# maxpit/human-pose-estimation

Measured on AMD Instinct MI355X. Metric: images/sec (224x224, batch 256/GPU), higher is better.
Workload: dtype f32; 1 GPU; batch=256/GPU 224x224x3 synthetic images, fp32 ResNet-50 v1 + 3-iter regressor + SMPL LBS at all 3 stages (configs[1] at batch 256; the BASELINE metric batch); global_batch=256, parallelism=dp1 (batch shard, replicated weights), regressor=synthetic 'survey' variant, input=float32 images resident in HBM

## Files before the change

human-pose-estimation_amd/_lib.py:

```python
from __future__ import annotations

import ctypes as C
import os

import numpy as np

_HERE = os.path.dirname(os.path.abspath(__file__))
LIB_PATH = os.path.join(_HERE, "lib", "libhpe_hip.so")

NUM_CONV = 53
NUM_DENSE = 3
NUM_CRITIC_DENSE = 9
NUM_VERTS = 6890
THETA_DIM = 85
FEATURE_DIM = 2048


class HpeError(RuntimeError):
    pass


class HpeConfig(C.Structure):
    _fields_ = [
        ("struct_size", C.c_int),
# ... 122 lines not shown
    r = HpeConvRoute(struct_size=C.sizeof(HpeConvRoute))
    check(lib.hpe_debug_conv_route(C.byref(cfg), int(idx), int(B), int(concurrent), int(residual), int(workspace), C.byref(r)))
    return r


ENCODER_PACKINGS = ("w", "w_split", "wino_u", "wino4_u", "stem_w", "scale", "shift", "w_dual", "w_dual_split", "shift_dual", "dxw", "flat")

OUTPUT_FIELDS = ("verts", "joints", "cams", "theta", "J_transformed", "kp2d", "verts2d", "Rs")


class HpeOutputs(C.Structure):
    _fields_ = [(n, C.c_void_p) for n in OUTPUT_FIELDS]


REDUCE_FN = C.CFUNCTYPE(C.c_int, C.c_void_p, C.c_void_p, C.c_longlong, C.c_void_p)

_PROTOS = {
    "hpe_last_error": (C.c_char_p, []),
    "hpe_version": (C.c_char_p, []),
    "hpe_conv_layer_name": (C.c_char_p, [C.c_int]),
    "hpe_bn_layer_name": (C.c_char_p, [C.c_int]),
    "hpe_conv_layer_geometry": (C.c_int, [C.c_int, C.POINTER(C.c_int)]),
    "hpe_config_init": (None, [C.POINTER(HpeConfig)]),
    "hpe_create": (C.c_int, [C.POINTER(HpeConfig), C.POINTER(C.c_void_p)]),
    "hpe_destroy": (C.c_int, [C.c_void_p]),
    "hpe_load_smpl": (C.c_int, [C.c_void_p, C.POINTER(HpeSmplModel)]),
    "hpe_load_conv": (C.c_int, [C.c_void_p, C.c_int] + [C.c_void_p] * 6),
    "hpe_load_dense": (C.c_int, [C.c_void_p, C.c_int, C.c_void_p, C.c_void_p]),
    "hpe_load_mean_theta": (C.c_int, [C.c_void_p, C.c_void_p]),
    "hpe_finalize": (C.c_int, [C.c_void_p]),
    "hpe_forward": (C.c_int, [C.c_void_p, C.c_void_p, C.c_int, C.POINTER(HpeOutputs), C.c_int, C.c_void_p]),
    "hpe_forward_pipelined": (C.c_int, [C.c_void_p, C.c_void_p, C.c_int, C.POINTER(HpeOutputs), C.c_int, C.c_void_p]),
    "hpe_join": (C.c_int, [C.c_void_p, C.c_void_p]),
    "hpe_tail": (C.c_int, [C.c_void_p, C.c_void_p, C.c_int, C.POINTER(HpeOutputs), C.c_int, C.c_void_p]),
    "hpe_tail_stream": (C.c_void_p, [C.c_void_p]),
    "hpe_encoder": (C.c_int, [C.c_void_p, C.c_void_p, C.c_int, C.c_void_p, C.c_void_p]),
    "hpe_regress_stage": (C.c_int, [C.c_void_p, C.c_void_p, C.c_void_p, C.c_int, C.c_void_p, C.c_void_p]),
    "hpe_smpl": (C.c_int, [C.c_void_p, C.c_void_p, C.c_int, C.POINTER(HpeOutputs), C.c_void_p]),
    "hpe_smpl_backward": (C.c_int, [C.c_void_p, C.c_void_p, C.c_int, C.POINTER(HpeOutputs), C.c_void_p, C.c_void_p]),
    "hpe_orth_proj": (C.c_int, [C.c_void_p, C.c_void_p, C.c_int, C.c_int, C.c_void_p, C.c_void_p]),
    "hpe_reproject_vertices": (C.c_int, [C.c_void_p, C.c_void_p, C.c_int, C.c_int, C.c_float, C.c_float, C.c_void_p, C.c_void_p]),
    "hpe_preprocess_u8": (C.c_int, [C.c_void_p, C.c_int, C.c_int, C.c_int, C.c_void_p, C.POINTER(C.c_int), C.c_void_p]),
    "hpe_preprocess_u8_batch": (C.c_int, [C.c_void_p, C.POINTER(C.c_longlong), C.POINTER(C.c_int), C.c_int, C.c_int, C.c_void_p, C.POINTER(C.c_int),
                                          C.c_void_p, C.c_void_p]),
    "hpe_augment_plan": (C.c_int, [C.c_int, C.c_void_p, C.c_void_p, C.c_void_p, C.c_void_p, C.c_void_p, C.c_int, C.c_void_p, C.c_void_p, C.c_void_p]),
    "hpe_augment_batch": (C.c_int, [C.c_void_p, C.c_void_p, C.c_void_p, C.c_void_p, C.c_void_p, C.c_int, C.c_void_p, C.c_void_p, C.c_void_p, C.c_void_p]),
    "hpe_adam_advance": (C.c_int, [C.c_void_p, C.c_double, C.c_double, C.c_double, C.c_void_p]),
    "hpe_adam_apply": (C.c_int, [C.c_void_p, C.c_void_p, C.c_void_p, C.c_void_p, C.c_longlong, C.c_void_p, C.c_float, C.c_float, C.c_float, C.c_void_p]),
    "hpe_adam_set_step": (C.c_int, [C.c_void_p, C.c_longlong, C.c_double, C.c_double, C.c_void_p]),
    "hpe_debug_adam_power": (C.c_int, [C.c_double, C.c_longlong, C.POINTER(C.c_double)]),
    "hpe_jpeg_info": (C.c_int, [C.c_int, C.c_void_p, C.c_void_p, C.c_void_p]),
    "hpe_jpeg_decode": (C.c_int, [C.c_int, C.c_void_p, C.c_void_p, C.c_void_p, C.c_int, C.c_void_p, C.c_longlong, C.c_void_p, C.c_void_p, C.c_void_p]),
    "hpe_jpeg_backend": (C.c_int, [C.c_void_p, C.c_void_p, C.c_int, C.c_void_p, C.c_longlong, C.c_void_p, C.c_longlong, C.c_void_p, C.c_longlong,
                                   C.c_void_p]),
    "hpe_jpeg_encode_layout": (C.c_int, [C.c_int, C.c_void_p, C.c_void_p, C.c_int, C.c_int, C.c_int, C.c_void_p, C.c_void_p]),
    "hpe_jpeg_forward": (C.c_int, [C.c_void_p, C.c_void_p, C.c_int, C.c_void_p, C.c_longlong, C.c_void_p, C.c_longlong, C.c_void_p]),
    "hpe_jpeg_entropy_encode": (C.c_int, [C.c_void_p, C.c_int, C.c_void_p, C.c_longlong, C.c_int, C.c_int, C.c_int, C.c_int, C.c_void_p, C.c_longlong,
                                          C.c_void_p, C.c_void_p]),
    "hpe_png_backend": (C.c_int, [C.c_void_p, C.c_void_p, C.c_int, C.c_void_p, C.c_longlong, C.c_void_p, C.c_longlong, C.c_void_p, C.c_longlong,
                                  C.c_void_p]),
    "hpe_png_filter": (C.c_int, [C.c_void_p, C.c_void_p, C.c_int, C.c_void_p, C.c_longlong, C.c_void_p, C.c_longlong, C.c_void_p]),
    "hpe_draw_panels": (C.c_int, [C.c_void_p] * 6 + [C.c_int, C.c_int, C.c_int, C.c_void_p, C.c_void_p]),
    "hpe_draw_skeleton": (C.c_int, [C.c_void_p] * 4 + [C.c_int, C.c_int, C.c_int, C.c_int, C.c_int, C.c_void_p]),
    "hpe_get_original": (C.c_int, [C.c_void_p, C.c_void_p, C.c_int, C.c_int, C.c_int, C.POINTER(C.c_int), C.c_float, C.c_int, C.c_void_p, C.POINTER(C.c_float), C.c_void_p, C.c_void_p, C.c_void_p]),
    "hpe_kp_loss": (C.c_int, [C.c_void_p, C.c_void_p, C.c_int, C.c_int, C.c_void_p, C.c_void_p]),
    "hpe_kp_loss_backward": (C.c_int, [C.c_void_p, C.c_void_p, C.c_int, C.c_int, C.c_void_p, C.c_void_p, C.c_void_p]),
    "hpe_mesh_loss": (C.c_int, [C.c_void_p, C.c_void_p, C.c_void_p, C.c_int, C.c_int, C.c_int, C.c_int, C.c_void_p, C.c_void_p]),
    "hpe_mesh_loss_grad": (C.c_int, [C.c_void_p, C.c_void_p, C.c_void_p, C.c_int, C.c_int, C.c_int, C.c_int, C.c_void_p, C.c_void_p, C.c_void_p,
                                     C.c_void_p, C.c_void_p]),
    "hpe_val_losses": (C.c_int, [C.c_void_p, C.c_void_p, C.c_void_p, C.POINTER(C.c_void_p), C.POINTER(C.c_void_p), C.c_int, C.c_int, C.c_int,
                                 C.c_int, C.c_int, C.c_int, C.c_void_p, C.c_void_p]),
    "hpe_eval_scores": (C.c_int, [C.POINTER(C.c_void_p), C.c_void_p, C.c_int, C.c_void_p, C.c_void_p, C.POINTER(C.c_void_p), C.c_int, C.c_int, C.c_int,
                                  C.c_int, C.c_int, C.c_int, C.c_void_p, C.c_void_p, C.c_void_p, C.c_void_p]),
    "hpe_critic_layer_name": (C.c_char_p, [C.c_int]),
    "hpe_critic_layer_shape": (C.c_int, [C.c_int, C.POINTER(C.c_int)]),
    "hpe_load_critic": (C.c_int, [C.c_void_p, C.POINTER(HpeCriticModel)]),
    "hpe_critic": (C.c_int, [C.c_void_p, C.c_void_p, C.c_int, C.c_void_p, C.c_int, C.c_void_p, C.c_int, C.c_void_p, C.c_void_p, C.c_void_p]),
    "hpe_critic_backward": (C.c_int, [C.c_void_p, C.c_void_p, C.c_int, C.c_void_p, C.c_int, C.c_void_p, C.c_int, C.c_void_p, C.c_void_p,
                                      C.c_void_p, C.c_void_p, C.c_void_p, C.c_void_p]),
    "hpe_critic_param_floats": (C.c_int, []),
    "hpe_critic_param_offset": (C.c_int, [C.c_int, C.c_int]),
    "hpe_critic_weight_grad_ws_floats": (C.c_longlong, [C.c_int]),
    "hpe_critic_reserve": (C.c_int, [C.c_void_p, C.c_int]),
    "hpe_critic_weight_grad": (C.c_int, [C.c_void_p, C.c_void_p, C.c_int, C.c_void_p, C.c_int, C.c_void_p, C.c_int, C.c_void_p, C.c_void_p,
                                         C.c_void_p, C.c_void_p, C.c_void_p, C.c_int, C.c_void_p, C.c_void_p]),
    "hpe_critic_get_params": (C.c_int, [C.c_void_p, C.c_void_p, C.c_void_p]),
    "hpe_critic_set_params_dev": (C.c_int, [C.c_void_p, C.c_void_p, C.c_void_p]),
    "hpe_regressor_param_floats": (C.c_int, []),
    "hpe_regressor_param_offset": (C.c_int, [C.c_int, C.c_int]),
    "hpe_regressor_get_params": (C.c_int, [C.c_void_p, C.c_void_p, C.c_void_p]),
    "hpe_regressor_set_params_dev": (C.c_int, [C.c_void_p, C.c_void_p, C.c_void_p]),
    "hpe_regressor_forward_train": (C.c_int, [C.c_void_p, C.c_void_p, C.c_int, C.c_void_p, C.c_void_p, C.c_void_p]),
    "hpe_regressor_backward": (C.c_int, [C.c_void_p, C.c_void_p, C.c_int, C.c_void_p, C.c_void_p, C.c_void_p, C.c_void_p, C.c_void_p]),
    "hpe_encoder_param_floats": (C.c_int, []),
    "hpe_encoder_param_offset": (C.c_int, [C.c_int, C.c_int]),
    "hpe_encoder_train_reserve": (C.c_int, [C.c_void_p, C.c_int]),
    "hpe_encoder_train_ws_floats": (C.c_longlong, [C.c_int]),
    "hpe_encoder_wg_slices": (C.c_int, [C.c_int, C.c_int]),
    "hpe_encoder_forward_train": (C.c_int, [C.c_void_p, C.c_void_p, C.c_int, C.c_void_p, C.c_void_p]),
    "hpe_encoder_backward": (C.c_int, [C.c_void_p, C.c_void_p, C.c_int, C.c_void_p, C.c_void_p, C.c_void_p]),
    "hpe_encoder_get_params": (C.c_int, [C.c_void_p, C.c_void_p, C.c_void_p]),
    "hpe_encoder_set_params": (C.c_int, [C.c_void_p, C.c_void_p]),
    "hpe_encoder_set_params_dev": (C.c_int, [C.c_void_p, C.c_void_p, C.c_void_p]),
    "hpe_debug_encoder_packing_bytes": (C.c_longlong, [C.c_void_p, C.c_int, C.c_int]),
    "hpe_debug_encoder_packing": (C.c_int, [C.c_void_p, C.c_int, C.c_int, C.c_void_p, C.c_void_p]),
    "hpe_debug_conv_backward": (C.c_int, [C.c_void_p, C.c_int, C.c_void_p, C.c_void_p, C.c_void_p, C.c_int, C.c_void_p, C.c_void_p, C.c_void_p]),
    "hpe_debug_maxpool_backward": (C.c_int, [C.c_void_p, C.c_void_p, C.c_int, C.c_int, C.c_int, C.c_void_p, C.c_void_p]),
    "hpe_debug_avgpool_backward": (C.c_int, [C.c_void_p, C.c_int, C.c_int, C.c_int, C.c_void_p, C.c_void_p]),
    "hpe_debug_encoder_stash": (C.c_int, [C.c_void_p, C.c_int, C.c_void_p, C.c_void_p]),
    "hpe_debug_encoder_stash_batch": (C.c_int, [C.c_void_p]),
    "hpe_encoder_train_reserve_mixed": (C.c_int, [C.c_void_p, C.c_int]),
    "hpe_encoder_train_ws_floats_mixed": (C.c_longlong, [C.c_int]),
    "hpe_encoder_forward_train_mixed": (C.c_int, [C.c_void_p, C.c_void_p, C.c_int, C.c_void_p, C.c_void_p]),
    "hpe_encoder_backward_mixed": (C.c_int, [C.c_void_p, C.c_void_p, C.c_int, C.c_void_p, C.c_void_p, C.c_void_p]),
    "hpe_debug_conv_backward_mixed": (C.c_int, [C.c_void_p, C.c_int, C.c_void_p, C.c_void_p, C.c_void_p, C.c_int, C.c_void_p, C.c_void_p, C.c_void_p]),
    "hpe_debug_maxpool_backward_mixed": (C.c_int, [C.c_void_p, C.c_void_p, C.c_int, C.c_int, C.c_int, C.c_void_p, C.c_void_p]),
    "hpe_debug_avgpool_backward_mixed": (C.c_int, [C.c_void_p, C.c_int, C.c_int, C.c_int, C.c_void_p, C.c_void_p]),
    "hpe_debug_encoder_stash_mixed": (C.c_int, [C.c_void_p, C.c_int, C.c_void_p, C.c_void_p]),
    "hpe_debug_encoder_stash_batch_mixed": (C.c_int, [C.c_void_p]),
    "hpe_encoder_stat_floats": (C.c_int, []),
    "hpe_encoder_stat_offset": (C.c_int, [C.c_int, C.c_int]),
    "hpe_encoder_train_reserve_batchnorm": (C.c_int, [C.c_void_p, C.c_int]),
    "hpe_encoder_train_ws_floats_batchnorm": (C.c_longlong, [C.c_int]),
    "hpe_debug_encoder_bn_slices": (C.c_int, [C.c_int, C.c_int]),
    "hpe_encoder_forward_batchnorm": (C.c_int, [C.c_void_p, C.c_void_p, C.c_int, C.c_void_p, C.c_void_p]),
    "hpe_encoder_backward_batchnorm": (C.c_int, [C.c_void_p, C.c_void_p, C.c_int, C.c_void_p, C.c_void_p, C.c_void_p]),
    "hpe_encoder_get_stats": (C.c_int, [C.c_void_p, C.c_void_p, C.c_void_p]),
    "hpe_encoder_update_stats": (C.c_int, [C.c_void_p, C.c_void_p, C.c_double, C.c_int, C.c_void_p]),
    "hpe_encoder_set_stats_dev": (C.c_int, [C.c_void_p, C.c_void_p, C.c_void_p]),
    "hpe_debug_conv_batchnorm": (C.c_int, [C.c_void_p, C.c_int, C.c_void_p, C.c_int, C.c_void_p, C.c_int, C.c_void_p, C.c_void_p, C.c_void_p, C.c_void_p]),
    "hpe_debug_conv_backward_batchnorm": (C.c_int, [C.c_void_p, C.c_int, C.c_void_p, C.c_void_p, C.c_void_p, C.c_void_p, C.c_int, C.c_void_p, C.c_void_p,
                                                    C.c_void_p]),
    "hpe_debug_encoder_stash_raw": (C.c_int, [C.c_void_p, C.c_int, C.c_void_p, C.c_void_p]),
    "hpe_debug_encoder_batch_stats": (C.c_int, [C.c_void_p, C.c_void_p, C.c_void_p]),
    "hpe_encoder_set_reduce": (C.c_int, [C.c_void_p, REDUCE_FN, C.c_void_p, C.c_int]),
    "hpe_debug_bn_sums": (C.c_int, [C.c_void_p, C.c_int, C.c_void_p, C.c_int, C.c_void_p, C.c_void_p]),
    "hpe_debug_bn_finish": (C.c_int, [C.c_void_p, C.c_int, C.c_void_p, C.c_longlong, C.c_void_p, C.c_int, C.c_void_p, C.c_int, C.c_void_p, C.c_void_p,
                                      C.c_void_p]),
    "hpe_debug_bn_backward_sums": (C.c_int, [C.c_void_p, C.c_int, C.c_void_p, C.c_void_p, C.c_void_p, C.c_int, C.c_void_p, C.c_longlong, C.c_void_p,
                                             C.c_void_p]),
    "hpe_debug_bn_backward_finish": (C.c_int, [C.c_void_p, C.c_int, C.c_void_p, C.c_void_p, C.c_void_p, C.c_void_p, C.c_int, C.c_void_p, C.c_void_p,
                                               C.c_longlong, C.c_void_p, C.c_void_p, C.c_void_p]),
    "hpe_device_status": (C.c_int, [C.c_void_p, C.c_void_p]),
    "hpe_debug_conv": (C.c_int, [C.c_void_p, C.c_int, C.c_void_p, C.c_int, C.c_void_p, C.c_int, C.c_void_p, C.c_void_p]),
    "hpe_debug_chain": (C.c_int, [C.c_void_p, C.c_int, C.c_void_p, C.c_void_p, C.c_int, C.c_void_p, C.c_void_p, C.POINTER(C.c_int), C.c_void_p]),
    "hpe_debug_stem": (C.c_int, [C.c_void_p, C.c_void_p, C.c_int, C.c_int, C.c_void_p, C.c_void_p]),
    "hpe_debug_gemm": (C.c_int, [C.c_void_p, C.c_void_p, C.c_void_p, C.c_int, C.c_int, C.c_int, C.c_int, C.c_int, C.c_void_p, C.c_int, C.c_void_p, C.c_void_p]),
    "hpe_debug_gemm_ex": (C.c_int, [C.c_void_p, C.POINTER(HpeDebugGemm), C.c_void_p]),
    "hpe_debug_gemm_check": (C.c_int, [C.POINTER(HpeDebugGemm), C.c_int, C.c_int]),
    "hpe_debug_gemm_launch": (C.c_int, [C.c_void_p, C.POINTER(HpeDebugGemm), C.c_int, C.c_int, C.c_void_p]),
    "hpe_debug_conv_route": (C.c_int, [C.POINTER(HpeConfig), C.c_int, C.c_int, C.c_int, C.c_int, C.c_int, C.POINTER(HpeConvRoute)]),
    "hpe_debug_conv_stream1x1": (C.c_int, [C.POINTER(HpeConfig), C.c_int, C.c_int, C.c_int, C.c_int]),
    "hpe_debug_dual": (C.c_int, [C.c_void_p, C.c_int, C.c_void_p, C.c_void_p, C.c_int, C.c_void_p, C.c_void_p]),
    "hpe_debug_maxpool": (C.c_int, [C.c_void_p, C.c_int, C.c_int, C.c_int, C.c_void_p, C.c_void_p]),
    "hpe_debug_avgpool": (C.c_int, [C.c_void_p, C.c_int, C.c_int, C.c_int, C.c_void_p, C.c_void_p]),
    "hpe_debug_joint_regress": (C.c_int, [C.c_void_p, C.c_void_p, C.c_int, C.c_int, C.c_void_p, C.c_void_p]),
    "hpe_enable_timing": (C.c_int, [C.c_void_p, C.c_int]),
    "hpe_get_timings": (C.c_int, [C.c_void_p, C.POINTER(C.c_float)]),
    "hpe_get_span_stats": (C.c_int, [C.c_void_p, C.POINTER(C.c_float), C.POINTER(C.c_int)]),
    "hpe_get_loss_timings": (C.c_int, [C.c_void_p, C.POINTER(C.c_float)]),
    "hpe_debug_set_loss_counter": (C.c_int, [C.c_void_p, C.c_void_p]),
    "hpe_get_conv_timings": (C.c_int, [C.c_void_p, C.POINTER(C.c_float)]),
    "hpe_render_params_init": (None, [C.POINTER(HpeRenderParams)]),
    "hpe_renderer_create": (C.c_int, [C.c_int, C.c_void_p, C.c_int, C.c_int, C.c_int, C.POINTER(C.c_void_p)]),
    "hpe_renderer_destroy": (C.c_int, [C.c_void_p]),
    "hpe_render": (C.c_int, [C.c_void_p, C.c_void_p, C.c_void_p, C.c_int, C.c_int, C.c_int, C.c_void_p, C.POINTER(HpeRenderParams), C.c_void_p,
                             C.c_void_p]),
    "hpe_debug_render_ids": (C.c_int, [C.c_void_p, C.c_void_p, C.c_void_p, C.c_int, C.c_int, C.c_int, C.POINTER(HpeRenderParams), C.c_void_p,
                                       C.c_void_p, C.c_void_p]),
    "hpe_debug_render_vertices": (C.c_int, [C.c_void_p, C.c_void_p, C.c_void_p, C.c_int, C.c_int, C.c_int, C.POINTER(HpeRenderParams),
                                            C.c_void_p, C.c_void_p]),
}

_lib = None


def load():
    global _lib
    if _lib is not None:
        return _lib
    if not os.path.exists(LIB_PATH):
        raise HpeError(
            "%s not found: build it with `python -c 'import __graft_entry__ as g; g.build()'` "
            "(hipcc --offload-arch=gfx950).  There is no CPU fallback." % LIB_PATH
        )
    try:
        import torch
    except Exception:
        pass
    lib = C.CDLL(LIB_PATH, mode=C.RTLD_GLOBAL)
    for name, (res, args) in _PROTOS.items():
        fn = getattr(lib, name)
        fn.restype = res
        fn.argtypes = args
    _lib = lib
    return lib


def declared_symbols():
    return sorted(_PROTOS)


def check(rc):
    if rc != 0:
        msg = load().hpe_last_error()
        raise HpeError("libhpe_hip error %d: %s" % (rc, msg.decode() if msg else "?"))


def f32(a):
    arr = np.ascontiguousarray(a, dtype=np.float32)
    return arr, arr.ctypes.data_as(C.c_void_p)
```

human-pose-estimation_amd/build.py:

```python
from __future__ import annotations

import os
import shutil
import subprocess
import sys

HERE = os.path.dirname(os.path.abspath(__file__))
CSRC = os.path.join(HERE, "csrc")
LIBDIR = os.path.join(HERE, "lib")
LIB = os.path.join(LIBDIR, "libhpe_hip.so")
SOURCES = ["conv_gemm.hip", "conv_gemm_f32s.hip", "conv_stream_f32s.hip", "conv_gemm_bf16.hip", "conv_gemm_bf16_p8.hip", "conv_chain_bf16.hip", "conv_chain_f32.hip", "conv3_halo_bf16.hip", "conv_wino.hip", "conv_wino4.hip", "stem_fused.hip", "encoder_ops.hip", "smpl.hip", "losses.hip", "prepost.hip", "render.hip", "hpe_plan.hip", "hpe_finalize.hip", "hpe_encoder.hip", "hpe_api.hip", "hpe_render_api.hip", "smpl_bwd.hip", "critic.hip", "critic_train.hip", "regressor_train.hip", "augment.hip", "encoder_train.hip", "encoder_grad.hip", "encoder_grad_bf16.hip", "encoder_repack.hip", "encoder_bn.hip", "jpeg_entropy.hip", "jpeg_decode.hip", "jpeg_huffman_enc.hip", "jpeg_encode.hip", "png_decode.hip", "png_encode.hip", "draw.hip", "adam.hip", "eval_scores.hip"]
CFLAGS = ["--offload-arch=gfx950", "-O3", "-std=c++17", "-fPIC", "-fvisibility=hidden", "-fno-fast-math"]


def _hipcc():
    for cand in (os.environ.get("HIPCC"), shutil.which("hipcc"), "/opt/rocm/bin/hipcc"):
        if cand and os.path.exists(cand):
            return cand
    raise RuntimeError("hipcc not found (set HIPCC or install ROCm under /opt/rocm)")


def _deps():
    return [os.path.join(CSRC, f) for f in os.listdir(CSRC) if f.endswith(".h")] + [os.path.join(HERE, "..", "include", "hpe.h")]


def _obj_stale(src, obj):
    if not os.path.exists(obj):
        return True
    t = os.path.getmtime(obj)
    return any(os.path.getmtime(d) > t for d in [src] + _deps() if os.path.exists(d))


def _flags_now():
    return " ".join(CFLAGS + os.environ.get("HPE_EXTRA_FLAGS", "").split())


def built_flags():
    tag = os.path.join(LIBDIR, "obj", "flags.txt")
    return open(tag).read() if os.path.exists(tag) else ""


def _stale():
    if not os.path.exists(LIB):
        return True
    if built_flags() != _flags_now():
        return True
    t = os.path.getmtime(LIB)
    deps = [os.path.join(CSRC, f) for f in os.listdir(CSRC)] + [os.path.join(HERE, "..", "include", "hpe.h")]
    return any(os.path.getmtime(d) > t for d in deps if os.path.exists(d))


def build(force=False, verbose=False):
    if not force and not _stale():
        return LIB
    os.makedirs(LIBDIR, exist_ok=True)
    objdir = os.path.join(LIBDIR, "obj")
    os.makedirs(objdir, exist_ok=True)
    extra = os.environ.get("HPE_EXTRA_FLAGS", "").split()
    tag = os.path.join(objdir, "flags.txt")
    flags_now = _flags_now()
    if force or not os.path.exists(tag) or open(tag).read() != flags_now:
        for f in os.listdir(objdir):
            os.remove(os.path.join(objdir, f))
    hipcc = _hipcc()
    jobs = []
    for s in SOURCES:
        src = os.path.join(CSRC, s)
        if not os.path.exists(src):
            continue
        obj = os.path.join(objdir, s.replace(".hip", ".o"))
        jobs.append((src, obj))

    def compile_one(job):
        src, obj = job
        if not _obj_stale(src, obj):
            return None
        cmd = [hipcc] + CFLAGS + extra + ["-c", "-o", obj + ".tmp%d" % os.getpid(), src]
        if verbose:
            print(" ".join(cmd), file=sys.stderr)
        r = subprocess.run(cmd, capture_output=True, text=True)
        if r.returncode != 0:
            return "hipcc failed on %s:\n%s%s" % (os.path.basename(src), r.stdout, r.stderr)
        os.replace(obj + ".tmp%d" % os.getpid(), obj)
        return None

    from concurrent.futures import ThreadPoolExecutor

    with ThreadPoolExecutor(max_workers=min(len(jobs), max(1, (os.cpu_count() or 2) - 1))) as ex:
        errs = [e for e in ex.map(compile_one, jobs) if e]
    if errs:
        raise RuntimeError("\n".join(errs))
    open(tag, "w").write(flags_now)
    tmp = LIB + ".tmp%d" % os.getpid()
    cmd = [hipcc, "--offload-arch=gfx950", "-shared", "-fPIC", "-o", tmp] + [o for _, o in jobs]
    r = subprocess.run(cmd, capture_output=True, text=True)
    if r.returncode != 0:
        raise RuntimeError("link failed:\n" + r.stdout + r.stderr)
    os.replace(tmp, LIB)
    return LIB


if __name__ == "__main__":
    print(build(force="--force" in sys.argv, verbose=True))
```

human-pose-estimation_amd/csrc/conv_stream_f32s.hip:

```cpp
#include <hip/hip_runtime.h>
#include <stdint.h>

#include "bf16_split.h"
#include "conv_gemm_common.h"
#include "gemm_contract.h"
#include "hpe_internal.h"
#include "lds_dma.h"

namespace {

constexpr int SBM = 32, SBN = 128, SNW = 4;

template <int K, bool DUAL>
__global__ __launch_bounds__(64 * SNW, 2) void conv_stream_f32s_kernel(GemmArgs p, int walkers) {
    constexpr bool RES = !DUAL;
    constexpr int NRES = RES ? SBM / (64 * SNW / (SBN / 4)) : 0;
    constexpr int KS = K / 16;
    constexpr int CH = K / 8;
    constexpr int RAW_BYTES = SBM * K * 4;
    constexpr int PLANE_BYTES = SBM * K * 2;
    constexpr int EP_BYTES = SBM * (SBN + 4) * 4;
    constexpr int WORK_BYTES = 3 * PLANE_BYTES > EP_BYTES ? 3 * PLANE_BYTES : EP_BYTES;
    constexpr int AP = RAW_BYTES / 1024 / SNW;
    constexpr int UN = SBM * CH / (64 * SNW);
    constexpr int NPASS = SBM / (64 * SNW / (SBN / 4));
    static_assert(K == 64 || K == 128, "K = 64 or 128");
    static_assert(!DUAL || K == 128, "dual: two sources of 64");
    static_assert(AP >= 1 && UN >= 1 && NPASS == 4, "tile geometry");

    __shared__ __attribute__((aligned(16))) float lds[WORK_BYTES / 4];
    __shared__ __attribute__((aligned(16))) float raw_lds[2 * RAW_BYTES / 4];
    char* const work = reinterpret_cast<char*>(lds);
    char* const raw = reinterpret_cast<char*>(raw_lds);

    const int bid = blockIdx.x;
    const int j = bid >> 3;
    const int slice = j % p.n_ntiles;
    const int walker = (j / p.n_ntiles) * 8 + (bid & 7);
    if (walker >= walkers || walker >= p.n_mtiles) return;
    const int n0 = slice * SBN;
    const int cnt = (p.n_mtiles - walker + walkers - 1) / walkers;

    const int t = threadIdx.x;
    const int lane = t & 63;
    const int wave = __builtin_amdgcn_readfirstlane(t >> 6);
    const int hi = lane >> 5;

    bf16x8 wreg[KS][3];
    {
        const __bf16* wsrc = reinterpret_cast<const __bf16*>(p.w) + (size_t)(n0 + 32 * wave + (lane & 31)) * p.ldw + 8 * hi;
#pragma unroll
        for (int q = 0; q < KS; ++q)
#pragma unroll
            for (int pc = 0; pc < 3; ++pc) wreg[q][pc] = *reinterpret_cast<const bf16x8*>(wsrc + pc * p.w_piece + 16 * q);
    }
    const int ncol = n0 + 32 * wave + (lane & 31);
    const float sc0 = p.scale[ncol], sh0 = p.shift[ncol];

    int dma_row[AP], dma_col[AP];
#pragma unroll
    for (int i = 0; i < AP; ++i) {
        const int s = (SNW * i + wave) * 64 + lane;
        dma_row[i] = s / (K / 4);
        dma_col[i] = (s % (K / 4)) * 4;
    }
    int sp_src[UN], sp_dst[UN];
#pragma unroll
    for (int u = 0; u < UN; ++u) {
        const int un = t + 64 * SNW * u;
        const int r = un / CH, c = un % CH;
        sp_src[u] = r * (K * 4) + c * 32;
        sp_dst[u] = r * (K * 2) + ((c ^ ((r / (16 / CH)) & (CH - 1))) << 4);
    }
    const int a_row = (lane & 31) * (K * 2);
    const int a_x = ((lane & 31) / (16 / CH)) & (CH - 1);
    const int r_row = t >> 5;
    const float* const res_col = RES ? p.res + n0 + (t & 31) * 4 : nullptr;

    auto issue_tile = [&](int m0, int buf, f32x4 (&rnext)[NPASS]) {
        asm volatile("" ::: "memory");
#pragma unroll
        for (int i = 0; i < AP; ++i) {
            int m = m0 + dma_row[i];
            m = m < p.M ? m : p.M - 1;
            const float* src = p.x + ((size_t)m * p.lda + dma_col[i]);
            if (DUAL && dma_col[i] >= 64) src = p.x2 + ((size_t)m * p.Cin + (dma_col[i] - 64));
            dma16(src, raw + buf * RAW_BYTES + (SNW * i + wave) * 1024);
        }
        asm volatile("" ::: "memory");
#pragma unroll
        for (int pass = 0; pass < NRES; ++pass) {
            int m = m0 + pass * 8 + r_row;
            m = m < p.M ? m : p.M - 1;
            rnext[pass] = HPE_RES_LOAD(reinterpret_cast<const f32x4*>(res_col + (size_t)m * p.ldres));
        }
        asm volatile("" ::: "memory");
    };

    auto tile_step = [&](int k, int buf, f32x4 (&rcur)[NPASS], f32x4 (&rnext)[NPASS]) {
        const int m0 = (walker + k * walkers) * SBM;
        const int m0n = k + 1 < cnt ? m0 + walkers * SBM : m0;
        wait_counts<NRES + NPASS>();
        bare_barrier();
        const unsigned rb = (unsigned)(uintptr_t)(const __attribute__((address_space(3))) char*)(raw + buf * RAW_BYTES);
#pragma unroll
        for (int u = 0; u < UN; ++u) {
            f32x4 lo, up;
            asm volatile("ds_read_b128 %0, %2\n\tds_read_b128 %1, %2 offset:16\n\ts_waitcnt lgkmcnt(0)" : "=&v"(lo), "=&v"(up) : "v"(rb + sp_src[u]) : "memory");
            bf16x8 h0, h1, h2;
            bf16_split3_cast<8>([&](int e) { return e < 4 ? lo[e] : up[e - 4]; }, h0, h1, h2);
            *reinterpret_cast<bf16x8*>(work + sp_dst[u]) = h0;
            *reinterpret_cast<bf16x8*>(work + PLANE_BYTES + sp_dst[u]) = h1;
            *reinterpret_cast<bf16x8*>(work + 2 * PLANE_BYTES + sp_dst[u]) = h2;
        }
        lds_barrier();
        issue_tile(m0n, buf ^ 1, rnext);

        f32x16 acc[1][1], acx;
#pragma unroll
        for (int e = 0; e < 16; ++e) acc[0][0][e] = acx[e] = 0.f;
#pragma unroll
        for (int q = 0; q < KS; ++q) {
            const int off = a_row + (((2 * q + hi) ^ a_x) << 4);
            const bf16x8 a0 = *reinterpret_cast<const bf16x8*>(work + off);
            const bf16x8 a1 = *reinterpret_cast<const bf16x8*>(work + PLANE_BYTES + off);
            const bf16x8 a2 = *reinterpret_cast<const bf16x8*>(work + 2 * PLANE_BYTES + off);
            acx = __builtin_amdgcn_mfma_f32_32x32x16_bf16(a2, wreg[q][0], acx, 0, 0, 0);
            acx = __builtin_amdgcn_mfma_f32_32x32x16_bf16(a1, wreg[q][1], acx, 0, 0, 0);
            acx = __builtin_amdgcn_mfma_f32_32x32x16_bf16(a0, wreg[q][2], acx, 0, 0, 0);
            acx = __builtin_amdgcn_mfma_f32_32x32x16_bf16(a1, wreg[q][0], acx, 0, 0, 0);
            acx = __builtin_amdgcn_mfma_f32_32x32x16_bf16(a0, wreg[q][1], acx, 0, 0, 0);
            acc[0][0] = __builtin_amdgcn_mfma_f32_32x32x16_bf16(a0, wreg[q][0], acc[0][0], 0, 0, 0);
        }
        acc[0][0] += acx;
        wait_counts<AP + NRES, 0>();
        bare_barrier();
        conv_epilogue<SBM, SBN, 1, SNW, true>(p, lds, acc, m0, n0, t, lane, 0, wave, rcur, RES, sc0, sh0);
    };

    f32x4 ra[NPASS], rb[NPASS];
    issue_tile(walker * SBM, 0, ra);
    wait_counts<0>();
    for (int k = 0; k < cnt; k += 2) {
        tile_step(k, 0, ra, rb);
        if (k + 1 < cnt) tile_step(k + 1, 1, rb, ra);
    }
    wait_counts<0>();
}

int device_cus() {
    static int n = 0;
    if (n == 0) {
        int dev = 0, v = 0;
        if (hipGetDevice(&dev) == hipSuccess && hipDeviceGetAttribute(&v, hipDeviceAttributeMultiprocessorCount, dev) == hipSuccess && v > 0) n = v;
        else n = 256;
    }
    return n;
}

}

bool hpe_stream_f32s_supported(int M, int N, int K) { return M > 0 && (K == 64 || K == 128) && N >= SBN && N % SBN == 0; }

bool hpe_stream_f32s_dual_supported(int M, int N, int K1, int K2, int stride, int Hi, int Ho) {
    return K1 == 64 && K2 == 64 && stride == 1 && Hi == Ho && hpe_stream_f32s_supported(M, N, K1 + K2);
}

hipError_t hpe_launch_stream_f32s(GemmArgs p, int mode, int max_walkers, hipStream_t st) {
    if ((mode != GEMM_DENSE && mode != GEMM_DUAL) || gemm_contract(p, mode, TILE_128x128, GEMM_K_F32S) || !hpe_stream_f32s_supported(p.M, p.N, p.K))
        return hipErrorInvalidValue;
    if (mode == GEMM_DENSE ? !p.res : (p.res || !hpe_stream_f32s_dual_supported(p.M, p.N, p.k1_slabs * BK, p.Cin, p.stride, p.Hi, p.Ho) || p.Wi != p.Wo))
        return hipErrorInvalidValue;
    p.n_mtiles = (p.M + SBM - 1) / SBM;
    p.n_ntiles = p.N / SBN;
    p.split_k = 1;
    p.res_prefetch = 1;
    int walkers = 2 * device_cus() / p.n_ntiles;
    if (max_walkers > 0 && walkers > max_walkers) walkers = max_walkers;
    if (walkers > p.n_mtiles) walkers = p.n_mtiles;
    if (walkers < 1) walkers = 1;
    const int grid = 8 * p.n_ntiles * ((walkers + 7) / 8);
    if (mode == GEMM_DUAL) hipLaunchKernelGGL((conv_stream_f32s_kernel<128, true>), dim3(grid), dim3(64 * SNW), 0, st, p, walkers);
    else if (p.K == 64) hipLaunchKernelGGL((conv_stream_f32s_kernel<64, false>), dim3(grid), dim3(64 * SNW), 0, st, p, walkers);
    else hipLaunchKernelGGL((conv_stream_f32s_kernel<128, false>), dim3(grid), dim3(64 * SNW), 0, st, p, walkers);
    return hipGetLastError();
}
```

human-pose-estimation_amd/csrc/hpe_api.hip:

```cpp
#include <hip/hip_runtime.h>

#include <algorithm>
#include <cmath>
#include <cstdint>
#include <cstdio>
#include <cstdlib>
#include <cstring>
#include <string>
#include <vector>

#include "gemm_contract.h"
#include "hpe_ctx.h"

namespace {
thread_local std::string g_err;
}

int fail(int code, const std::string& msg) {
    g_err = msg;
    return code;
}

int check_ready(hpe_ctx* c, int B, int need) {
    if (!c) return fail(HPE_ERR_INVALID, "null ctx");
// ... 655 lines not shown
    GemmArgs p{};
    p.x = g->x, p.x2 = g->x2, p.w = g->wt, p.res = g->residual, p.y = g->y;
    p.M = g->M, p.N = g->N, p.K = g->K;
    p.lda = g->lda, p.ldw = g->ldw, p.ldy = g->ldy, p.ldres = g->ldres, p.w_rows = g->w_rows;
    p.Hi = g->Hi, p.Wi = g->Wi, p.Cin = g->Cin, p.Ho = g->Ho, p.Wo = g->Wo, p.stride = g->stride;
    p.cin_slabs = g->Cin / slab;
    p.k1_slabs = g->k1_slabs;
    p.relu = g->relu;
    p.y_slab8 = g->y_slab8;
    return p;
}

static std::string debug_gemm_refusal(const HpeDebugGemm* g) {
    if (!g) return "null HpeDebugGemm";
    if (g->struct_size != (int)sizeof(HpeDebugGemm))
        return "HpeDebugGemm.struct_size is " + std::to_string(g->struct_size) + ", this library's is " + std::to_string(sizeof(HpeDebugGemm)) +
               " (other revision of include/hpe.h?)";
    if (g->mode != HPE_GEMM_DENSE && g->mode != HPE_GEMM_STRIDED && g->mode != HPE_GEMM_CONV3 && g->mode != HPE_GEMM_DUAL)
        return "HpeDebugGemm.mode must be dense, strided, conv3 or dual";
    return "";
}

static std::string debug_gemm_rejected(const HpeDebugGemm* g, const char* clause) {
    return "mode " + std::to_string(g->mode) + " tile " + std::to_string(g->tile) + " M " + std::to_string(g->M) + " N " + std::to_string(g->N) + " K " +
           std::to_string(g->K) + " is outside the launcher's contract (gemm_contract.h), clause \"" + clause + "\": nothing was launched";
}

int hpe_debug_gemm_ex(hpe_ctx* c, const HpeDebugGemm* g, void* stream) {
    if (g && g->split_k) *g->split_k = 0;
    if (!c || !c->finalized) return fail(HPE_ERR_STATE, "needs a finalized ctx");
    const std::string why = debug_gemm_refusal(g);
    if (!why.empty()) return fail(HPE_ERR_INVALID, why);
    if ((!g->scale || !g->shift) && g->N > 1024) return fail(HPE_ERR_INVALID, "hpe_debug_gemm_ex: N <= 1024 without scale / shift");
    DeviceGuard guard(c->cfg.device);
    GemmArgs p = debug_gemm_args(g, 32);
    p.scale = g->scale ? g->scale : c->ones;
    p.shift = g->shift ? g->shift : c->zeros;
    p.zero = c->zeros;
    if (g->use_splitk) {
        p.partial = c->partial;
        p.partial_floats = c->partial_floats;
    }
    if (const char* clause = gemm_contract(p, g->mode, g->tile, GEMM_K_F32)) return fail(HPE_ERR_INVALID, "hpe_debug_gemm_ex: " + debug_gemm_rejected(g, clause));
    int split_k = 0;
    const hipError_t e = hpe_launch_gemm(p, g->mode, g->tile, c->plan.splitk_min_slabs, static_cast<hipStream_t>(stream), &split_k);
    if (g->split_k) *g->split_k = split_k;
    if (e == hipErrorInvalidValue && split_k == 0) return fail(HPE_ERR_INVALID, "hpe_debug_gemm_ex: the launcher refused the plan's splitk_min_slabs, nothing was launched");
    HIP_TRY(e);
    return HPE_OK;
}

int hpe_debug_gemm_check(const HpeDebugGemm* g, int kernel, int w_piece) {
    const std::string why = debug_gemm_refusal(g);
    if (!why.empty()) return fail(HPE_ERR_INVALID, why);
    if (kernel < GEMM_K_F32 || kernel > GEMM_K_BF16_P8) return fail(HPE_ERR_INVALID, "hpe_debug_gemm_check: kernel must be 0 (fp32), 1 (f32s), 2 (bf16) or 3 (bf16_p8)");
    const GemmKernel k = static_cast<GemmKernel>(kernel);
    GemmArgs p = debug_gemm_args(g, gemm_rules(k).slab);
    alignas(16) static const float present[4] = {};
    p.scale = p.shift = p.zero = present;
    if (k == GEMM_K_F32S) p.w_piece = w_piece;
    if (const char* clause = gemm_contract(p, g->mode, g->tile, k)) return fail(HPE_ERR_INVALID, "hpe_debug_gemm_check: " + debug_gemm_rejected(g, clause));
    return HPE_OK;
}

int hpe_debug_gemm_launch(hpe_ctx* c, const HpeDebugGemm* g, int kernel, int w_piece, void* stream) {
    if (kernel == GEMM_K_F32) return hpe_debug_gemm_ex(c, g, stream);
    if (g && g->split_k) *g->split_k = 0;
    const std::string why = debug_gemm_refusal(g);
    if (!why.empty()) return fail(HPE_ERR_INVALID, why);
    if (kernel < GEMM_K_F32 || kernel > GEMM_K_BF16_P8) return fail(HPE_ERR_INVALID, "hpe_debug_gemm_launch: kernel must be 0 (fp32), 1 (f32s), 2 (bf16) or 3 (bf16_p8)");
    if ((!g->scale || !g->shift) && g->N > 1024) return fail(HPE_ERR_INVALID, "hpe_debug_gemm_launch: N <= 1024 without scale / shift");
    const GemmKernel k = static_cast<GemmKernel>(kernel);
    GemmArgs p = debug_gemm_args(g, gemm_rules(k).slab);
    if (k == GEMM_K_F32S) p.w_piece = w_piece;
    alignas(16) static const float present[4] = {};
    p.scale = g->scale ? g->scale : present;
    p.shift = g->shift ? g->shift : present;
    p.zero = present;
    if (const char* clause = gemm_contract(p, g->mode, g->tile, k)) return fail(HPE_ERR_INVALID, "hpe_debug_gemm_launch: " + debug_gemm_rejected(g, clause));
    if (!c || !c->finalized) return fail(HPE_ERR_STATE, "needs a finalized ctx");
    DeviceGuard guard(c->cfg.device);
    p.scale = g->scale ? g->scale : c->ones;
    p.shift = g->shift ? g->shift : c->zeros;
    p.zero = c->zeros;
    if (g->use_splitk) {
        p.partial = c->partial;
        p.partial_floats = c->partial_floats;
    }
    if (const char* clause = gemm_contract(p, g->mode, g->tile, k)) return fail(HPE_ERR_INVALID, "hpe_debug_gemm_launch: " + debug_gemm_rejected(g, clause));
    int split_k = 1;
    hipStream_t st = static_cast<hipStream_t>(stream);
    const hipError_t e = k == GEMM_K_F32S ? hpe_launch_gemm_f32s(p, g->mode, g->tile, st)
                       : k == GEMM_K_BF16 ? hpe_launch_gemm_bf16(p, g->mode, g->tile, st)
                                          : hpe_launch_gemm_bf16_p8(p, g->mode, st, &split_k);
    if (g->split_k) *g->split_k = split_k;
    HIP_TRY(e);
    return HPE_OK;
}

int hpe_debug_conv_route(const HpeConfig* cfg, int idx, int B, int concurrent, int residual, int workspace, HpeConvRoute* out) {
    static_assert(HPE_CONV_K_F32 == CONV_K_F32 && HPE_CONV_K_HALO3 == CONV_K_HALO3 && HPE_CONV_K_WINO4_FUSED == CONV_K_WINO4_FUSED && HPE_CONV_K_COUNT == CONV_K_WINO4_FUSED + 1,
                  "include/hpe.h numbers the kernels as ConvKernel does");
    if (!cfg || !out) return fail(HPE_ERR_INVALID, "null argument");
    if (cfg->struct_size != (int)sizeof(HpeConfig) || out->struct_size != (int)sizeof(HpeConvRoute))
        return fail(HPE_ERR_INVALID, "hpe_debug_conv_route: HpeConfig.struct_size / HpeConvRoute.struct_size are " + std::to_string(cfg->struct_size) + " / " +
                                         std::to_string(out->struct_size) + ", this library's are " + std::to_string(sizeof(HpeConfig)) + " / " + std::to_string(sizeof(HpeConvRoute)));
    if (idx < 0 || idx >= HPE_NUM_CONV || B < 1) return fail(HPE_ERR_INVALID, "hpe_debug_conv_route: idx must be in [0, HPE_NUM_CONV) and B >= 1");
    const HpePlan pl = hpe_resolve_plan(*cfg);
    const bool bf16 = cfg->encoder_dtype == 1;
    const ConvQuery q{B, concurrent != 0, residual != 0, workspace != 0};
    const ConvRoute r = route_conv(pl, bf16, idx, q);
    *out = HpeConvRoute{(int)sizeof(HpeConvRoute), r.kernel, r.mode, r.tile, r.in_slab8, 0, 0, -1, -1, 0, layer_packs(pl, bf16, idx), 0};
    for (const ResBlock& blk : blocks()) {
        if (idx != blk.i2a && idx != blk.i2c) continue;
        const BlockRoute b = route_block(pl, bf16, blk, q);
        if (idx == blk.i2a) out->out_slab8 = b.r2a.out_slab8;
        if (idx == blk.i2c) out->join = b.join, out->next_slab8 = b.u1_slab8;
        if (idx == blk.i2c && b.join == JOIN_DUAL) out->join_kernel = b.r2c.kernel, out->join_tile = b.r2c.tile;
    }
    return HPE_OK;
}

int hpe_debug_conv_stream1x1(const HpeConfig* cfg, int idx, int B, int concurrent, int residual) {
    if (!cfg || cfg->struct_size != (int)sizeof(HpeConfig) || idx < 0 || idx >= HPE_NUM_CONV || B < 1) {
        fail(HPE_ERR_INVALID, "hpe_debug_conv_stream1x1: cfg (struct_size), idx in [0, HPE_NUM_CONV) and B >= 1");
        return -1;
    }
    const HpePlan pl = hpe_resolve_plan(*cfg);
    const bool bf16 = cfg->encoder_dtype == 1;
    const ConvQuery q{B, concurrent != 0, residual != 0, true};
    for (const ResBlock& blk : blocks())
        if (blk.first && blk.i2c == idx) {
            const BlockRoute b = route_block(pl, bf16, blk, q);
            return (stream1x1_dual(pl, bf16, blk) ? 2 : 0) | (b.join == JOIN_DUAL && b.r2c.stream ? 1 : 0);
        }
    return (stream1x1_layer(pl, bf16, idx) ? 2 : 0) | (route_conv(pl, bf16, idx, q).stream ? 1 : 0);
}

int hpe_debug_dual(hpe_ctx* c, int idx2c, const float* t2, const float* x, int B, float* y, void* stream) {
    int rc = check_ready(c, B, NEED_ENC);
    if (rc) return rc;
    if (!t2 || !x || !y || c->bf16) return fail(HPE_ERR_INVALID, "hpe_debug_dual: null pointer, or a bf16 context");
    for (const ResBlock& blk : blocks()) {
        if (!blk.first || blk.i2c != idx2c) continue;
        const BlockRoute b = route_block(c->plan, false, blk, ConvQuery{B, false, false, c->wino_v != nullptr});
        if (b.join != JOIN_DUAL) break;
        DeviceGuard g(c->cfg.device);
        HIP_TRY(run_dual(c, blk.i2c, blk.i1, b.r2c, t2, x, B, y, static_cast<hipStream_t>(stream)));
        return HPE_OK;
    }
    return fail(HPE_ERR_INVALID, "hpe_debug_dual: idx2c must be the branch2c of a conv_block that this plan runs as the dual-source launch");
}

int hpe_debug_gemm(hpe_ctx* c, const float* x, const float* wt, int M, int N, int K, int w_rows, int tile, const float* residual,
                   int relu, float* y, void* stream) {
    if (!c || !c->finalized || !c->have_regressor) return fail(HPE_ERR_STATE, "needs a finalized ctx with the regressor loaded");
    if (!x || !wt || !y || N > 1024) return fail(HPE_ERR_INVALID, "bad argument (N <= 1024)");
    HpeDebugGemm g{};
    g.struct_size = (int)sizeof(HpeDebugGemm);
    g.mode = HPE_GEMM_DENSE;
    g.tile = tile;
    g.x = x;
    g.wt = wt;
    g.residual = residual;
    g.y = y;
    g.M = M;
    g.N = N;
    g.K = K;
    g.lda = K;
    g.ldw = K;
    g.w_rows = w_rows;
    g.ldy = N;
    g.ldres = N;
    g.relu = relu;
    g.use_splitk = 0;
    return hpe_debug_gemm_ex(c, &g, stream);
}

int hpe_debug_maxpool(const float* x, int B, int H, int C, float* y, void* stream) {
    if (!x || !y || B < 1) return fail(HPE_ERR_INVALID, "bad argument");
    HIP_TRY(hpe_launch_maxpool(x, y, B, H, C, static_cast<hipStream_t>(stream)));
    return HPE_OK;
}

int hpe_debug_avgpool(const float* x, int B, int HW, int C, float* y, void* stream) {
    if (!x || !y || B < 1) return fail(HPE_ERR_INVALID, "bad argument");
    HIP_TRY(hpe_launch_avgpool(x, y, B, HW, C, C, static_cast<hipStream_t>(stream)));
    return HPE_OK;
}

int hpe_debug_joint_regress(hpe_ctx* c, const float* X, int n, int use_kp, float* out, void* stream) {
    if (!c || !c->finalized || !c->have_smpl) return fail(HPE_ERR_STATE, "SMPL not finalized");
    if (!X || !out || n < 1) return fail(HPE_ERR_INVALID, "bad argument");
    DeviceGuard g(c->cfg.device);
    HIP_TRY(hpe_launch_joint_regress(X, use_kp ? c->smpl.kp_reg : c->smpl.j_reg, n, use_kp ? c->num_kp : 24, out, nullptr, nullptr,
                                     static_cast<hipStream_t>(stream)));
    return HPE_OK;
}

int hpe_device_status(hpe_ctx* c, void* stream) {
    if (!c || !c->finalized) return fail(HPE_ERR_STATE, "needs a finalized ctx");
    DeviceGuard g(c->cfg.device);
    HIP_TRY(hipStreamSynchronize(static_cast<hipStream_t>(stream)));
    if (c->dev_err) {
        unsigned w = 0;
        HIP_TRY(hipMemcpy(&w, c->dev_err, sizeof w, hipMemcpyDeviceToHost));
        if (w) {
            (void)hipMemset(c->dev_err, 0, sizeof w);
            return fail(HPE_ERR_HIP, "device error word " + std::to_string(w) +
                                         ": a stream-K wait of the Winograd GEMM timed out, outputs since the last check are invalid");
        }
    }
    return HPE_OK;
}

int hpe_enable_timing(hpe_ctx* c, int enable) {
    if (!c) return fail(HPE_ERR_INVALID, "null ctx");
    c->timing = enable;
    c->span_n = 0;
    c->timed_valid = false;
    c->conv_timed_valid = false;
    return HPE_OK;
}

int hpe_get_timings(hpe_ctx* c, float ms[5]) {
    if (!c || !ms) return fail(HPE_ERR_INVALID, "null argument");
    if (!c->timed_valid) return fail(HPE_ERR_STATE, "no timed call recorded (hpe_enable_timing first)");
    DeviceGuard g(c->cfg.device);
    HIP_TRY(hipEventSynchronize(c->ev[4]));
    for (int i = 0; i < 5; ++i) ms[i] = 0.f;
    HIP_TRY(hipEventElapsedTime(&ms[0], c->ev[0], c->ev[1]));
    HIP_TRY(hipEventElapsedTime(&ms[4], c->ev[0], c->ev[4]));
    if (c->conv_timed_valid) {
        for (int i = 0; i < HPE_NUM_CONV; ++i) {
            float t = 0.f;
            HIP_TRY(hipEventElapsedTime(&t, c->cev0[i], c->cev1[i]));
            ms[1] += t;
        }
    }
    ms[2] = ms[4] - ms[0];
    return HPE_OK;
}

int hpe_get_span_stats(hpe_ctx* c, float ms[3], int* n_calls) {
    if (!c || !ms || !n_calls) return fail(HPE_ERR_INVALID, "null argument");
    if (c->span_n == 0) return fail(HPE_ERR_STATE, "no timed call recorded (hpe_enable_timing first)");
    DeviceGuard g(c->cfg.device);
    const unsigned n = c->span_n < (unsigned)hpe_ctx::SPAN_RING ? c->span_n : (unsigned)hpe_ctx::SPAN_RING;
    double sum = 0.0;
    float lo = 1e30f, hi = 0.f;
    for (unsigned i = 0; i < n; ++i) {
        float t = 0.f;
        HIP_TRY(hipEventSynchronize(c->span1[i]));
        HIP_TRY(hipEventElapsedTime(&t, c->span0[i], c->span1[i]));
        sum += t;
        lo = t < lo ? t : lo;
        hi = t > hi ? t : hi;
    }
    ms[0] = (float)(sum / n);
    ms[1] = lo;
    ms[2] = hi;
    *n_calls = (int)n;
    return HPE_OK;
}

int hpe_get_loss_timings(hpe_ctx* c, float ms[2]) {
    if (!c || !ms) return fail(HPE_ERR_INVALID, "null argument");
    if (c->loss_timed_stages == 0) return fail(HPE_ERR_STATE, "no timed hpe_val_losses call recorded (hpe_enable_timing first)");
    DeviceGuard g(c->cfg.device);
    HIP_TRY(hipEventSynchronize(c->lev_all[1]));
    HIP_TRY(hipEventElapsedTime(&ms[0], c->lev_all[0], c->lev_all[1]));
    ms[1] = 0.f;
    for (int s = 0; s < c->loss_timed_stages; ++s) {
        float t = 0.f;
        HIP_TRY(hipEventElapsedTime(&t, c->lev0[s], c->lev1[s]));
        ms[1] += t;
    }
    return HPE_OK;
}

int hpe_debug_set_loss_counter(hpe_ctx* c, void* counter_dev) {
    if (!c) return fail(HPE_ERR_INVALID, "null ctx");
    c->loss_counter = static_cast<unsigned long long*>(counter_dev);
    return HPE_OK;
}

int hpe_get_conv_timings(hpe_ctx* c, float* ms) {
    if (!c || !ms) return fail(HPE_ERR_INVALID, "null argument");
    if (!c->conv_timed_valid) return fail(HPE_ERR_STATE, "no level-2 timed call recorded");
    DeviceGuard g(c->cfg.device);
    HIP_TRY(hipEventSynchronize(c->ev[4]));
    for (int i = 0; i < HPE_NUM_CONV; ++i) HIP_TRY(hipEventElapsedTime(&ms[i], c->cev0[i], c->cev1[i]));
    return HPE_OK;
}

}
#pragma GCC visibility pop
```

human-pose-estimation_amd/csrc/hpe_ctx.h:

```cpp
#pragma once
#include <hip/hip_runtime.h>

#include <cmath>
#include <cstdint>
#include <cstring>
#include <string>
#include <vector>

#include "../../include/hpe.h"
#include "bf16_split.h"
#include "hpe_internal.h"
#include "hpe_plan.h"

int fail(int code, const std::string& msg);

#define HIP_TRY(expr)                                                                                             \
    do {                                                                                                          \
        hipError_t _e = (expr);                                                                                   \
        if (_e != hipSuccess)                                                                                     \
            return fail(HPE_ERR_HIP, std::string(#expr) + ": " + hipGetErrorString(_e) + " (" __FILE__ ":" +      \
                                         std::to_string(__LINE__) + ")");                                         \
    } while (0)

struct ConvSpec {
// ... 129 lines not shown
    size_t partial_floats = 0;
    float *dsh = nullptr;
    float *wgp = nullptr;
    float *zeros = nullptr;
    float *feat = nullptr;
    float *dxw[HPE_NUM_CONV] = {};
    int bn_B = 0;
    int bn_stat_B = 0;
    float *zstash = nullptr;
    float *bn_batch = nullptr;
    float *bn_stats = nullptr;
    double *bn_part = nullptr;
    int *bn_hw = nullptr;
    hpe_reduce_fn reduce = nullptr;
    void *reduce_user = nullptr;
    int reduce_G = 0;
    int reduce_failed = -1;
    int bn_stat_G = 0;
    int mx_B = 0;
    int mx_stash_B = 0;
    unsigned short *mx_stash = nullptr;
    unsigned short *mx_g0 = nullptr, *mx_g1 = nullptr, *mx_sbig = nullptr, *mx_t0 = nullptr, *mx_t1 = nullptr, *mx_ssmall = nullptr;
    unsigned short *mx_padded = nullptr;
    unsigned short *mx_w[HPE_NUM_CONV] = {};
    unsigned short *mx_dxw[HPE_NUM_CONV] = {};
    void *mx_cast = nullptr;
};
constexpr int MX_CAST_SEGS = 2 * HPE_NUM_CONV - 1;
struct MxCastSeg {
    const float* src;
    unsigned short* dst;
    int src_pitch, dst_pitch;
    long quads;
};
constexpr int BN_MAX_SLICES = 512;
constexpr int BN_PART_COLS = 262144;
constexpr int WG_MAX_SLICES = 128;
constexpr int WG_WGP_FLOATS = 1152 * 512;
static_assert(WG_WGP_FLOATS >= 3 * 2 * 2048, "the reduce buffers of data-parallel training fit the weight gradient's scratch");
inline size_t conv_dxw_floats(int idx) {
    const ConvSpec& s = specs()[idx];
    return idx == 0 ? 0 : (size_t)round_up(s.cin, 128) * s.kh * s.kw * s.cout;
}
struct EncLayout {
    int off[HPE_NUM_CONV][4];
    int stat[HPE_NUM_CONV];
    size_t stash[HPE_NUM_CONV];
    size_t stash_pool, stash_per_image;
    int total, channels;
};
const EncLayout& layout();

struct hpe_ctx {
    HpeConfig cfg{};
    bool finalized = false;
    bool dead = false;
    HpePlan plan;
    bool bf16 = false;
    bool have_encoder = false, have_regressor = false, have_smpl = false;
    ConvLayer conv[HPE_NUM_CONV];
    DenseLayer dense[HPE_NUM_DENSE];
    bool smpl_loaded = false, mean_loaded = false;
    std::vector<float> h_vt, h_sd, h_pd, h_jreg, h_w, h_kreg;
    std::vector<int> h_par;
    int num_kp = 19;
    float h_mean[HPE_THETA_DIM];
    float *w1f = nullptr, *w1t = nullptr, *w2 = nullptr, *w3 = nullptr, *b1 = nullptr, *b2 = nullptr, *b3 = nullptr;
    float *ones = nullptr, *zeros = nullptr, *mean_dev = nullptr;
    EncTrainWork et{};
    RegTrainWork rt{};
    SmplDev smpl{};
    SmplWork work{};
    SmplBwdWork bwd{};
    float* smpl_basis_src = nullptr;
    float *padded = nullptr, *X0 = nullptr, *X1 = nullptr, *T1 = nullptr, *T2 = nullptr, *SC = nullptr;
    float *feat = nullptr, *P1 = nullptr, *H1 = nullptr, *H2 = nullptr, *thA = nullptr, *thB = nullptr;
    float* critic_buf = nullptr;
    CriticW critic{};
    bool have_critic = false;
    float* critic_ws = nullptr;
    size_t critic_ws_floats = 0;
    float* loss_ws = nullptr;
    size_t loss_ws_floats = 0;
    std::vector<void*> allocs;
    float* partial = nullptr;
    size_t partial_floats = 0;
    float* wino_v = nullptr;
    float* wino_ws = nullptr;
    unsigned* wino_flags = nullptr;
    unsigned* dev_err = nullptr;
    unsigned wino_epoch = 0;
    int n_cu = 0;
    bool loss_attr_done = false;
    unsigned long long* loss_counter = nullptr;
    hipStream_t aux[3]{};
    hipEvent_t ev_fork{}, ev_join[3]{};
    hipStream_t tail_st{};
    hipEvent_t ev_enc{}, ev_tail{}, ev_feat_free[2]{};
    bool feat_free_valid[2] = {false, false};
    bool tail_pending = false;
    unsigned pipe_idx = 0;
    float* feat_alt = nullptr;
    int co_running = 1;
    float* w4_split = nullptr;
    float* partial_tail = nullptr;
    size_t partial_tail_floats = 0;
    bool dense_on_tail = false;
    int timing = 0;
    hipEvent_t ev[8]{};
    static constexpr int SPAN_RING = 64;
    hipEvent_t span0[SPAN_RING]{}, span1[SPAN_RING]{};
    unsigned span_n = 0;
    hipEvent_t cev0[HPE_NUM_CONV]{}, cev1[HPE_NUM_CONV]{};
    hipEvent_t lev0[16]{}, lev1[16]{}, lev_all[2]{};
    int loss_timed_stages = 0;
    bool ev_ok = false, timed_valid = false, conv_timed_valid = false;
};

struct DeviceGuard {
    int prev = -1;
    bool changed = false;
    explicit DeviceGuard(int dev) {
        if (hipGetDevice(&prev) == hipSuccess && prev != dev) changed = hipSetDevice(dev) == hipSuccess;
    }
    ~DeviceGuard() {
        if (changed) (void)hipSetDevice(prev);
    }
};

int dev_alloc(hpe_ctx* c, float** p, size_t n_floats, bool zero);
int upload(hpe_ctx* c, float** p, const std::vector<float>& h);
int upload_split(hpe_ctx* c, void** p, const std::vector<float>& wt, int rows, int K);

#define HIPE(expr)                               \
    do {                                         \
        hipError_t _e = (expr);                  \
        if (_e != hipSuccess) return _e;         \
    } while (0)

enum { NEED_ENC = 1, NEED_REG = 2, NEED_SMPL = 4 };
int check_ready(hpe_ctx* c, int B, int need);

int finalize_impl(hpe_ctx* c);
void release_device_state(hpe_ctx* c);
int repack_encoder(hpe_ctx* c);

hipError_t run_conv(hpe_ctx* c, int idx, const ConvRoute& r, const float* x, int B, const float* res, int relu, float* y, hipStream_t st,
                    float* wino_v = nullptr, int slot = 0, const float* scale = nullptr, const float* shift = nullptr);
hipError_t run_dual(hpe_ctx* c, int i2c, int i1, const ConvRoute& r, const float* t2, const float* x, int B, float* y, hipStream_t st);
hipError_t run_conv_nhwc(hpe_ctx* c, int idx, const float* x, int B, const float* res, int relu, float* y, hipStream_t st,
                         const float* scale = nullptr, const float* shift = nullptr);
hipError_t run_chain(hpe_ctx* c, int i2c, bool first, const float* t2, const float* res, int B, float* t3, float* u1, hipStream_t st,
                     bool u1_slab8 = false);
hipError_t encoder_impl(hpe_ctx* c, const float* images, int B, float* features, int ldfeat, hipStream_t st);
hipError_t run_dense(hpe_ctx* c, const float* x, int lda, int M, int K, const float* w, int w_rows, int N, const float* scale, const float* shift,
                     const float* res, int ldres, int relu, float* y, int ldy, hipStream_t st, float* partial = nullptr, size_t partial_floats = 0);
hipError_t regress_impl(hpe_ctx* c, const float* th_prev, float* th_next, int B, hipStream_t st);
hipError_t features_proj(hpe_ctx* c, const float* features, int B, hipStream_t st);
hipError_t tail_impl(hpe_ctx* c, const float* feat, int B, const HpeOutputs* stage_outs, int n_outs, hipStream_t ts, hipEvent_t feat_free);
hipError_t join_tail(hpe_ctx* c, hipStream_t st);
int forward_impl(hpe_ctx* c, const float* images, int B, const HpeOutputs* stage_outs, int n_outs, hipStream_t st, bool pipelined);

size_t encoder_repack_reserve_floats();
int encoder_repack_reserve(hpe_ctx* c);
hipError_t encoder_repack_launch(hpe_ctx* c, const float* flat_dev, hipStream_t st);

hipError_t encoder_repack_stats_launch(hpe_ctx* c, hipStream_t st);

int bn_slices(int M, int N);
hipError_t bn_launch_stats(const float* z, int M, int N, float eps, double* part, float* mu, float* var, float* r, hipStream_t st);
hipError_t bn_launch_apply(const float* z, const float* mu, const float* r, const float* gamma, const float* beta, const float* res, int relu, float* y,
                           int M, int N, hipStream_t st);
hipError_t bn_launch_bwd_reduce(const float* dy, const float* y, const float* z, const float* mu, const float* r, int M, int N, double* part, float* db,
                                float* dgamma, float* dbeta, hipStream_t st);
hipError_t bn_launch_bwd_apply(const float* dy, const float* y, const float* z, const float* mu, const float* r, const float* gamma, const float* dgamma,
                               const float* dbeta, int M, int N, float* dz, float* dzraw, hipStream_t st, double M_all = 0.0);
hipError_t bn_launch_stats_sums(const float* z, int M, int N, double* part, double* sums, hipStream_t st);
hipError_t bn_launch_stats_from_sums(const double* sums, double M_all, int N, float eps, float* mu, float* var, float* r, hipStream_t st);
hipError_t bn_launch_bwd_sums(const float* dy, const float* y, const float* z, const float* mu, const float* r, int M, int N, double* part, double* sums,
                              float* db, float* dgamma, float* dbeta, hipStream_t st);
hipError_t bn_launch_bwd_from_sums(const double* sums, int N, float* red, hipStream_t st);
hipError_t bn_launch_momentum(float* stats, const float* batch, const int* hw, int B, int channels, double momentum, int unbiased, hipStream_t st);
hipError_t bn_launch_install(const float* stats, int channels, float eps, float* keep, float* mean, float* istd, double* sd, hipStream_t st);

void wg_slicing(int idx, int B, int* P, int* slices);
size_t wg_partial_floats(int B);
void gate(const float* dy, const float* y, const float* s, float* dz, float* dzs, long n, int N, hipStream_t st);
hipError_t weight_grad(hpe_ctx* c, int idx, const float* x, const float* dz, int B, float* grad_layer, hipStream_t st, bool bn = false);
hipError_t data_grad(hpe_ctx* c, int idx, const float* dzs, int B, const float* res, float* out, hipStream_t st);
void scatter2(const float* lo, float* hi, int B, int H, int C, hipStream_t st);
void avgpool_bwd(const float* dy, float* dx, int B, int HW, int C, hipStream_t st);
void maxpool_bwd(const float* x, const float* dy, float* dx, int B, int H, int C, hipStream_t st);

void wg_slicing16(int idx, int B, int* P, int* slices);
hipError_t wg_finish(hpe_ctx* c, int idx, int n_kc, int slices, float* grad_layer, hipStream_t st);

typedef unsigned short* mx16;
typedef const unsigned short* cmx16;
hipError_t mx_cast_launch(hpe_ctx* c, int first, int segs, hipStream_t st);
hipError_t mx_conv_forward(hpe_ctx* c, int idx, cmx16 x, int B, cmx16 res, int relu, mx16 y, hipStream_t st);
void mx_gate(cmx16 dy, cmx16 y, const float* s, mx16 dz, mx16 dzs, long n, int N, hipStream_t st);
hipError_t mx_weight_grad(hpe_ctx* c, int idx, cmx16 x, cmx16 dz, int B, float* grad_layer, hipStream_t st);
hipError_t mx_data_grad(hpe_ctx* c, int idx, cmx16 dzs, int B, cmx16 res, mx16 out, hipStream_t st);
void mx_scatter2(cmx16 lo, mx16 hi, int B, int H, int C, hipStream_t st);
void mx_avgpool_bwd(const float* dy, mx16 dx, int B, int HW, int C, hipStream_t st);
void mx_maxpool_bwd(cmx16 x, cmx16 dy, mx16 dx, int B, int H, int C, hipStream_t st);

int regressor_param_offset(int idx, bool bias);
hipError_t regressor_train_forward(hpe_ctx* c, const float* features, int B, const float* drop, hipStream_t st);
hipError_t regressor_train_backward(hpe_ctx* c, const float* features, int B, const float* drop, const float* grad_thetas, float* grad_flat,
                                    float* grad_features, hipStream_t st);
hipError_t regressor_params_copy(hpe_ctx* c, float* flat, bool set, hipStream_t st);
```

human-pose-estimation_amd/csrc/hpe_encoder.hip:

```cpp
#include <hip/hip_runtime.h>

#include <cmath>
#include <cstdint>
#include <cstdio>
#include <cstdlib>
#include <cstring>
#include <string>
#include <vector>

#include "hpe_ctx.h"

static hipError_t launch_gemm(hpe_ctx* c, GemmArgs& p, const ConvRoute& r, const void* w_split, hipStream_t st) {
    if (!r.concurrent) p.partial = c->partial, p.partial_floats = c->partial_floats;
    if (r.kernel == CONV_K_BF16 || r.kernel == CONV_K_BF16_P8) return hpe_launch_gemm_bf16(p, r.mode, r.tile, st);
    if (r.kernel != CONV_K_F32S) return hpe_launch_gemm(p, r.mode, r.tile, c->plan.splitk_min_slabs, st);
    if (!w_split) return hipErrorInvalidValue;
    p.w = static_cast<const float*>(w_split);
    p.w_piece = p.ldw;
    p.ldw *= 3;
    return hpe_launch_gemm_f32s(p, r.mode, r.tile, st);
}

hipError_t run_conv(hpe_ctx* c, int idx, const ConvRoute& r, const float* x, int B, const float* res, int relu, float* y, hipStream_t st,
                    float* wino_v, int slot, const float* scale, const float* shift) {
    const ConvSpec& s = specs()[idx];
    const ConvLayer& L = c->conv[idx];
    if (!scale) scale = L.scale;
    if (!shift) shift = L.shift;
    const int H = s.hin;
    const bool f2 = r.kernel == CONV_K_WINO || r.kernel == CONV_K_WINO_FUSED, f4 = r.kernel == CONV_K_WINO4 || r.kernel == CONV_K_WINO4_FUSED;
    if ((r.kernel >= CONV_K_HALO3 && res) || (f2 && !L.wino_u) || (f4 && !L.wino4_u) || ((f2 || f4) && !r.in_slab8 && !wino_v)) return hipErrorInvalidValue;
    switch (r.kernel) {
        case CONV_K_WINO4_FUSED: return hpe_launch_wino4_fused_conv3(x, L.wino4_u, scale, shift, c->zeros, y, s.cout, B, H, H, s.cin, s.cout, relu, st);
        case CONV_K_WINO_FUSED: return hpe_launch_wino_fused_conv3(x, L.wino_u_split, scale, shift, c->zeros, y, s.cout, B, H, H, s.cin, s.cout, relu, st);
        case CONV_K_WINO4:
            return hpe_launch_wino4_conv3(x, s.cin, L.wino4_u, scale, shift, y, s.cout, B, H, H, s.cin, s.cout, relu, wino_v, st, r.concurrent ? c->co_running : 1,
                                          c->w4_split && slot >= 0 && slot < 4 ? c->w4_split + (size_t)slot * hpe_wino4_split_ws_floats() : nullptr, c->plan.wino4_n32,
                                          c->plan.w4_abl);
        case CONV_K_WINO: {
            WinoStreamK sk{};
            if (c->wino_ws && slot >= 0 && slot < 4) {
                sk.ws = c->wino_ws + (size_t)slot * c->n_cu * HPE_WINO_WS_FLOATS;
                sk.flags = c->wino_flags + (size_t)slot * c->n_cu;
                sk.epoch = ++c->wino_epoch;
                if (sk.epoch == 0) sk.epoch = ++c->wino_epoch;
                sk.n_wg = c->n_cu;
                sk.err = c->dev_err;
            }
            return hpe_launch_wino_conv3(x, s.cin, L.wino_u, scale, shift, y, s.cout, B, H, H, s.cin, s.cout, relu, wino_v, c->wino_ws ? &sk : nullptr, st);
        }
        case CONV_K_HALO3: {
            Halo3Args h{};
            h.x = reinterpret_cast<const __bf16*>(x), h.w = reinterpret_cast<const __bf16*>(L.w), h.y = reinterpret_cast<__bf16*>(y);
            h.scale = scale, h.shift = shift;
            h.M = B * s.hout * s.hout, h.N = s.cout, h.ldw = L.k_pad;
            h.relu = relu, h.two = c->plan.halo3_two;
            return hpe_launch_halo3_bf16(h, H, s.cin, st);
        }
    }
    GemmArgs p{};
    p.x = x, p.w = L.w, p.scale = scale, p.shift = shift, p.res = res, p.y = y, p.zero = c->zeros;
    p.M = B * s.hout * s.hout, p.N = s.cout, p.K = L.k_pad;
    p.lda = s.cin, p.ldw = L.k_pad, p.w_rows = L.n_pad, p.ldy = p.ldres = s.cout;
    p.Hi = p.Wi = H, p.Cin = s.cin, p.Ho = p.Wo = s.hout, p.stride = s.stride;
    p.cin_slabs = s.cin / (c->bf16 ? 64 : 32);
    p.relu = relu, p.y_slab8 = r.out_slab8 ? 1 : 0;
    if (r.mode == GEMM_STEM) p.Hi = STEM_HP, p.Wi = STEM_WP, p.Cin = 4;
    if (r.stream) {
        if (!L.w_stream || !res) return hipErrorInvalidValue;
        p.w = reinterpret_cast<const float*>(L.w_stream);
        p.w_piece = p.ldw;
        p.ldw *= 3;
        return hpe_launch_stream_f32s(p, GEMM_DENSE, c->plan.stream1x1_walkers, st);
    }
    return launch_gemm(c, p, r, L.w_split, st);
}

hipError_t run_conv_nhwc(hpe_ctx* c, int idx, const float* x, int B, const float* res, int relu, float* y, hipStream_t st, const float* scale,
                         const float* shift) {
    const ConvRoute r = route_conv(c->plan, c->bf16, idx, ConvQuery{B, false, res != nullptr, c->wino_v != nullptr});
    if (r.in_slab8) {
        const ConvSpec& s = specs()[idx];
        HIPE(hpe_launch_nhwc_to_slab8(x, c->T1, (long)B * s.hin * s.hin, s.cin, st));
        x = c->T1;
    }
    return run_conv(c, idx, r, x, B, res, relu, y, st, c->wino_v, 0, scale, shift);
}

hipError_t run_dual(hpe_ctx* c, int i2c, int i1, const ConvRoute& r, const float* t2, const float* x, int B, float* y, hipStream_t st) {
    const ConvSpec& s2 = specs()[i2c];
    const ConvSpec& s1 = specs()[i1];
    const ConvLayer& L = c->conv[i2c];
    GemmArgs p{};
    p.x = t2, p.x2 = x, p.w = L.w_dual, p.scale = c->ones, p.shift = L.shift_dual, p.y = y, p.zero = c->zeros;
    p.M = B * s2.hout * s2.hout, p.N = s2.cout, p.K = L.k_dual;
    p.k1_slabs = L.k1_dual / (c->bf16 ? 64 : 32), p.relu = 1;
    p.lda = s2.cin, p.ldw = L.k_dual, p.w_rows = round_up(s2.cout, 128), p.ldy = s2.cout;
    p.Hi = p.Wi = s1.hin, p.Cin = s1.cin, p.Ho = p.Wo = s1.hout, p.stride = s1.stride;
    if (r.stream) {
        if (!L.w_dual_stream) return hipErrorInvalidValue;
        p.w = reinterpret_cast<const float*>(L.w_dual_stream);
        p.w_piece = p.ldw;
        p.ldw *= 3;
        return hpe_launch_stream_f32s(p, GEMM_DUAL, c->plan.stream1x1_walkers, st);
    }
    return launch_gemm(c, p, r, L.w_dual_split, st);
}

hipError_t run_chain(hpe_ctx* c, int i2c, bool first, const float* t2, const float* res, int B, float* t3, float* u1, hipStream_t st,
                     bool u1_slab8) {
    const ConvSpec& s2 = specs()[i2c];
    const int inext = i2c + (first ? 2 : 1);
    const ConvSpec& sn = specs()[inext];
    const ConvLayer& L2 = c->conv[i2c];
    const ConvLayer& Ln = c->conv[inext];
    if (!c->bf16) {
        ChainArgsF32 q{};
        q.t2 = t2;
        q.res = res;
        q.w2c = L2.w;
        q.w2a = Ln.w;
        q.scaleA = L2.scale;
        q.shiftA = L2.shift;
        q.scaleB = Ln.scale;
        q.shiftB = Ln.shift;
        q.t3 = t3;
        q.u1 = u1;
        q.M = B * s2.hout * s2.hout;
        q.ldw2c = L2.k_pad;
        q.ldw2a = Ln.k_pad;
        q.u1_slab8 = u1_slab8 ? 1 : 0;
        return hpe_launch_chain_f32(q, s2.cin, s2.cout, sn.cout, st);
    }
    ChainArgs p{};
    p.t2 = reinterpret_cast<const __bf16*>(t2);
    if (first) {
        p.x2 = reinterpret_cast<const __bf16*>(res);
        p.w2c = reinterpret_cast<const __bf16*>(L2.w_dual);
        p.scaleA = c->ones;
        p.shiftA = L2.shift_dual;
        p.ldw2c = L2.k_dual;
    } else {
        p.res = reinterpret_cast<const __bf16*>(res);
        p.w2c = reinterpret_cast<const __bf16*>(L2.w);
        p.scaleA = L2.scale;
        p.shiftA = L2.shift;
        p.ldw2c = L2.k_pad;
    }
    p.w2a = reinterpret_cast<const __bf16*>(Ln.w);
    p.scaleB = Ln.scale;
    p.shiftB = Ln.shift;
    p.t3 = reinterpret_cast<__bf16*>(t3);
    p.u1 = reinterpret_cast<__bf16*>(u1);
    p.M = B * s2.hout * s2.hout;
    p.ldw2a = Ln.k_pad;
    return hpe_launch_chain_bf16(p, s2.cin, s2.cout, sn.cout, first ? specs()[i2c + 1].cin : 0, st);
}

hipError_t run_dense(hpe_ctx* c, const float* x, int lda, int M, int K, const float* w, int w_rows, int N, const float* scale,
                     const float* shift, const float* res, int ldres, int relu, float* y, int ldy, hipStream_t st, float* partial,
                     size_t partial_floats) {
    if (M <= 4) return hpe_launch_dense_gemv(x, lda, M, K, w, N, scale, shift, res, ldres, relu, y, ldy, st);
    GemmArgs p{};
    p.zero = shift;
    p.partial = partial ? partial : c->dense_on_tail ? c->partial_tail : c->partial;
    p.partial_floats = partial ? partial_floats : c->dense_on_tail ? c->partial_tail_floats : c->partial_floats;
    p.x = x;
    p.w = w;
    p.scale = scale;
    p.shift = shift;
    p.res = res;
    p.y = y;
    p.M = M;
    p.N = N;
    p.K = K;
    p.lda = lda;
    p.ldw = K;
    p.w_rows = w_rows;
    p.ldy = ldy;
    p.ldres = ldres;
    p.relu = relu;
    return hpe_launch_gemm(p, GEMM_DENSE, TILE_64x64, c->plan.splitk_min_slabs, st);
}

static hipError_t timed_conv(hpe_ctx* c, int idx, const ConvRoute& r, const float* x, int B, const float* res, int relu, float* y, hipStream_t st,
                             float* wino_v = nullptr, int slot = 0) {
    const bool t2 = c->timing >= 2;
    if (t2) HIPE(hipEventRecord(c->cev0[idx], st));
    HIPE(run_conv(c, idx, r, x, B, res, relu, y, st, wino_v, slot));
    if (t2) HIPE(hipEventRecord(c->cev1[idx], st));
    return hipSuccess;
}

static hipError_t encoder_chunk(hpe_ctx* c, const float* images, int i0, int B, float* features, int ldfeat, hipStream_t st, int slot = 0,
                         bool concurrent = false) {
    const int esz = c->bf16 ? 2 : 4;
    auto at = [&](float* base, size_t elems) { return reinterpret_cast<float*>(reinterpret_cast<char*>(base) + elems * esz); };
    const size_t o_img = (size_t)i0 * HPE_IMG_SIZE * HPE_IMG_SIZE * 3;
    const size_t o_pad = (size_t)i0 * STEM_HP * STEM_WP * 4;
    const size_t o_big = (size_t)i0 * 802816;
    const size_t o_mid = (size_t)i0 * 200704;
    float* padded = at(c->padded, o_pad);
    float* SC = at(c->SC, o_big);
    float* T1 = at(c->T1, o_mid);
    float* T2 = at(c->T2, o_mid);
    float* cur = at(c->X0, o_big);
    float* nxt = at(c->X1, o_big);
    float* wv = (c->wino_v && (i0 == 0 || B >= 32)) ? c->wino_v + (size_t)i0 * WINO_V_PITCH : nullptr;
    const ConvQuery q{B, concurrent, false, wv != nullptr};
    if (c->plan.stem_fused && (reinterpret_cast<uintptr_t>(images + o_img) & 15) == 0) {
        const bool t2 = c->timing >= 2;
        if (t2) HIPE(hipEventRecord(c->cev0[0], st));
        HIPE(hpe_launch_stem_fused(images + o_img, c->conv[0].stem_w, c->conv[0].scale, c->conv[0].shift, cur, B, hpe_stem_fused_pick_rows(B),
                                   c->bf16 ? 1 : 0, st));
        if (t2) HIPE(hipEventRecord(c->cev1[0], st));
    } else if (c->bf16) {
        HIPE(hpe_launch_pad_input_bf16(images + o_img, padded, B, HPE_IMG_SIZE, HPE_IMG_SIZE, STEM_HP, STEM_WP, st));
        HIPE(timed_conv(c, 0, route_conv(c->plan, true, 0, q), padded, B, nullptr, 1, SC, st));
        HIPE(hpe_launch_maxpool_bf16(SC, cur, B, 112, 64, st));
    } else {
        HIPE(hpe_launch_pad_input(images + o_img, padded, B, HPE_IMG_SIZE, HPE_IMG_SIZE, STEM_HP, STEM_WP, st));
        HIPE(timed_conv(c, 0, route_conv(c->plan, false, 0, q), padded, B, nullptr, 1, SC, st));
        HIPE(hpe_launch_maxpool(SC, cur, B, 112, 64, st));
    }
    bool have_2a = false;
    for (const ResBlock& blk : blocks()) {
        const bool first = blk.first;
        const int i2a = blk.i2a, i2b = blk.i2b, i2c = blk.i2c, i1 = blk.i1;
        const BlockRoute br = route_block(c->plan, c->bf16, blk, q);
        if (have_2a) {
            if (c->timing >= 2) {
                HIPE(hipEventRecord(c->cev0[i2a], st));
                HIPE(hipEventRecord(c->cev1[i2a], st));
            }
        } else {
            HIPE(timed_conv(c, i2a, br.r2a, cur, B, nullptr, 1, T1, st));
        }
        have_2a = false;
        HIPE(timed_conv(c, i2b, br.r2b, T1, B, nullptr, 1, T2, st, wv, slot));
        const float* res = cur;
        if (br.join == JOIN_CHAIN) {
            const bool t2 = c->timing >= 2;
            if (t2) HIPE(hipEventRecord(c->cev0[i2c], st));
            HIPE(run_chain(c, i2c, first, T2, cur, B, nxt, T1, st, br.u1_slab8));
            if (t2) {
                HIPE(hipEventRecord(c->cev1[i2c], st));
                if (first) {
                    HIPE(hipEventRecord(c->cev0[i1], st));
                    HIPE(hipEventRecord(c->cev1[i1], st));
                }
            }
            have_2a = true;
        } else if (br.join == JOIN_DUAL) {
            const bool t2 = c->timing >= 2;
            if (t2) HIPE(hipEventRecord(c->cev0[i2c], st));
            HIPE(run_dual(c, i2c, i1, br.r2c, T2, cur, B, nxt, st));
            if (t2) {
                HIPE(hipEventRecord(c->cev1[i2c], st));
                HIPE(hipEventRecord(c->cev0[i1], st));
                HIPE(hipEventRecord(c->cev1[i1], st));
            }
        } else {
            if (first) {
                HIPE(timed_conv(c, i1, br.r1, cur, B, nullptr, 0, SC, st));
                res = SC;
            }
            HIPE(timed_conv(c, i2c, br.r2c, T2, B, res, 1, nxt, st));
        }
        float* t = cur;
        cur = nxt;
        nxt = t;
    }
    if (c->bf16) return hpe_launch_avgpool_bf16(cur, features + (size_t)i0 * ldfeat, B, 49, HPE_FEATURE_DIM, ldfeat, st);
    return hpe_launch_avgpool(cur, features + (size_t)i0 * ldfeat, B, 49, HPE_FEATURE_DIM, ldfeat, st);
}

hipError_t encoder_impl(hpe_ctx* c, const float* images, int B, float* features, int ldfeat, hipStream_t st) {
    int nstream = c->plan.n_streams;
    if (nstream > B / c->plan.min_chunk) nstream = B / c->plan.min_chunk;
    if (c->timing >= 2 || nstream < 2) nstream = 1;
    if (nstream == 1) return encoder_chunk(c, images, 0, B, features, ldfeat, st);
    int nchunk = nstream;
    if (c->plan.chunk_images > 0) {
        const int want = c->plan.chunk_images < c->plan.min_chunk ? c->plan.min_chunk : c->plan.chunk_images;
        nchunk = B / want;
        if (nchunk < nstream) nchunk = nstream;
    }
    const int per = (B + nchunk - 1) / nchunk;
    nchunk = (B + per - 1) / per;
    HIPE(hipEventRecord(c->ev_fork, st));
    for (int k = 1; k < nstream; ++k) HIPE(hipStreamWaitEvent(c->aux[k - 1], c->ev_fork, 0));
    c->co_running = nstream;
    for (int k = 0; k < nchunk; ++k) {
        const int i0 = k * per;
        const int n = (i0 + per <= B) ? per : (B - i0);
        const int sid = k % nstream;
        hipStream_t s = (sid == 0) ? st : c->aux[sid - 1];
        const hipError_t ec = encoder_chunk(c, images, i0, n, features, ldfeat, s, sid, true);
        if (ec != hipSuccess) {
            c->co_running = 1;
            return ec;
        }
    }
    c->co_running = 1;
    for (int k = 1; k < nstream; ++k) {
        HIPE(hipEventRecord(c->ev_join[k - 1], c->aux[k - 1]));
        HIPE(hipStreamWaitEvent(st, c->ev_join[k - 1], 0));
    }
    return hipSuccess;
}

hipError_t regress_impl(hpe_ctx* c, const float* th_prev, float* th_next, int B, hipStream_t st) {
    HIPE(run_dense(c, th_prev, THETA_LD, B, THETA_LD, c->w1t, 1024, 1024, c->ones, c->b1, c->P1, 1024, 1, c->H1, 1024, st));
    HIPE(run_dense(c, c->H1, 1024, B, 1024, c->w2, 1024, 1024, c->ones, c->b2, nullptr, 0, 1, c->H2, 1024, st));
    return run_dense(c, c->H2, 1024, B, 1024, c->w3, 128, HPE_THETA_DIM, c->ones, c->b3, th_prev, THETA_LD, 0, th_next, THETA_LD, st);
}

hipError_t features_proj(hpe_ctx* c, const float* features, int B, hipStream_t st) {
    return run_dense(c, features, HPE_FEATURE_DIM, B, HPE_FEATURE_DIM, c->w1f, 1024, 1024, c->ones, c->zeros, nullptr, 0, 0, c->P1,
                     1024, st);
}

hipError_t tail_impl(hpe_ctx* c, const float* feat, int B, const HpeOutputs* stage_outs, int n_outs, hipStream_t ts, hipEvent_t feat_free) {
    hipError_t e = features_proj(c, feat, B, ts);
    if (e == hipSuccess && feat_free) e = hipEventRecord(feat_free, ts);
    if (e == hipSuccess) e = hpe_launch_tile_theta(c->mean_dev, c->thA, B, THETA_LD, ts);
    float* prev = c->thA;
    float* next = c->thB;
    const int first_out = c->cfg.num_stage - n_outs;
    for (int s = 0; e == hipSuccess && s < c->cfg.num_stage; ++s) {
        e = regress_impl(c, prev, next, B, ts);
        if (e == hipSuccess && s >= first_out) e = hpe_launch_smpl(c->smpl, c->work, next, THETA_LD, B, &stage_outs[s - first_out], ts);
        float* t = prev;
        prev = next;
        next = t;
    }
    return e;
}

hipError_t join_tail(hpe_ctx* c, hipStream_t st) {
    if (!c->tail_pending) return hipSuccess;
    HIPE(hipStreamWaitEvent(st, c->ev_tail, 0));
    c->tail_pending = false;
    return hipSuccess;
}

int forward_impl(hpe_ctx* c, const float* images, int B, const HpeOutputs* stage_outs, int n_outs, hipStream_t st, bool pipelined) {
    int rc = check_ready(c, B, NEED_ENC | NEED_REG | NEED_SMPL);
    if (rc) return rc;
    if (!images || !stage_outs) return fail(HPE_ERR_INVALID, "null pointer");
    if (n_outs < 1 || n_outs > c->cfg.num_stage) return fail(HPE_ERR_INVALID, "n_outs must be in [1, num_stage]");
    DeviceGuard g(c->cfg.device);
    const bool tm = c->timing != 0;
    if (c->timing >= 2) pipelined = false;
    float* feat = c->feat;
    hipStream_t ts = st;
    if (pipelined) {
        const unsigned slot = c->pipe_idx & 1u;
        feat = slot ? c->feat_alt : c->feat;
        if (c->feat_free_valid[slot]) HIP_TRY(hipStreamWaitEvent(st, c->ev_feat_free[slot], 0));
        ts = c->tail_st;
    } else {
        HIP_TRY(join_tail(c, st));
    }
    if (tm) {
        HIP_TRY(hipEventRecord(c->ev[0], st));
        HIP_TRY(hipEventRecord(c->span0[c->span_n % hpe_ctx::SPAN_RING], st));
    }
    HIP_TRY(encoder_impl(c, images, B, feat, HPE_FEATURE_DIM, st));
    if (tm) {
        HIP_TRY(hipEventRecord(c->ev[1], st));
        HIP_TRY(hipEventRecord(c->span1[c->span_n % hpe_ctx::SPAN_RING], st));
        ++c->span_n;
    }
    if (pipelined) {
        HIP_TRY(hipEventRecord(c->ev_enc, st));
        HIP_TRY(hipStreamWaitEvent(ts, c->ev_enc, 0));
        c->dense_on_tail = true;
    }
    hipEvent_t feat_free = nullptr;
    if (pipelined) {
        const unsigned slot = c->pipe_idx & 1u;
        feat_free = c->ev_feat_free[slot];
        c->feat_free_valid[slot] = true;
    }
    hipError_t e = tail_impl(c, feat, B, stage_outs, n_outs, ts, feat_free);
    c->dense_on_tail = false;
    if (e != hipSuccess) return fail(HPE_ERR_HIP, std::string("forward tail: ") + hipGetErrorString(e));
    if (pipelined) {
        HIP_TRY(hipEventRecord(c->ev_tail, ts));
        c->tail_pending = true;
        ++c->pipe_idx;
    }
    if (tm) {
// ... 8 lines not shown
```

human-pose-estimation_amd/csrc/hpe_internal.h:

```cpp
#pragma once
#include <hip/hip_runtime.h>
#include <stddef.h>

#include "../../include/hpe.h"

typedef float f32x4 __attribute__((ext_vector_type(4)));
typedef float f32x16 __attribute__((ext_vector_type(16)));

template <typename Id>
__device__ __forceinline__ int xcd_remap(Id bid, int total) {
    const int xcd = bid & 7;
    const int q = total >> 3, rr = total & 7;
    return (xcd < rr ? xcd * (q + 1) : rr * (q + 1) + (xcd - rr) * q) + (bid >> 3);
}

inline dim3 grid1(long n) { return dim3((unsigned)((n + 255) / 256)); }

enum GemmMode { GEMM_DENSE = 0, GEMM_STRIDED = 1, GEMM_CONV3 = 2, GEMM_STEM = 3, GEMM_DUAL = 4 };
enum GemmTile { TILE_128x128 = 0, TILE_128x64 = 1, TILE_64x64 = 2, TILE_64x128 = 3, TILE_128x128_W8 = 4, TILE_128x64_W8 = 5, TILE_256x128_W8 = 6,
                TILE_P8_256x256 = 7  };

struct GemmArgs {
    const float* x;
    const float* w;
    const float* scale;
    const float* shift;
    const float* res;
    float* y;
    int M, N, K;
    int lda, ldw, ldy, ldres, w_rows;
    int relu;
    int Hi, Wi, Cin, Ho, Wo, stride, cin_slabs;
    int n_mtiles, n_ntiles;
    int split_k;
    float* partial;
    size_t partial_floats;
    const float* zero;
    void* reserved;
    const float* x2;
    int k1_slabs;
    int res_prefetch;
    int y_slab8;
    int w_piece;
};

hipError_t hpe_launch_gemm(GemmArgs p, int mode, int tile, int splitk_min_slabs, hipStream_t st, int* split_k_out = nullptr);
hipError_t hpe_launch_gemm_f32s(GemmArgs p, int mode, int tile, hipStream_t st);
bool hpe_stream_f32s_supported(int M, int N, int K);
bool hpe_stream_f32s_dual_supported(int M, int N, int K1, int K2, int stride, int Hi, int Ho);
hipError_t hpe_launch_stream_f32s(GemmArgs p, int mode, int max_walkers, hipStream_t st);

size_t hpe_wino_v_floats(int B, int H, int W, int C);
hipError_t hpe_wino_init_device();
#define HPE_WINO_WS_FLOATS 65536
struct WinoStreamK {
    float* ws;
    unsigned* flags;
    unsigned epoch;
    int n_wg;
    unsigned* err;
};
hipError_t hpe_launch_wino_conv3(const float* x, int lda, const float* U, const float* scale, const float* shift, float* y, int ldy,
                                 int B, int H, int W, int C, int N, int relu, float* V, const WinoStreamK* sk, hipStream_t st);

hipError_t hpe_launch_wino_fused_conv3(const float* xs, const unsigned short* Us, const float* scale, const float* shift, const float* zero16, float* y,
                                       int ldy, int B, int H, int W, int C, int N, int relu, hipStream_t st);
int hpe_wino_fused_items(int B, int H, int W, int N);
hipError_t hpe_launch_nhwc_to_slab8(const float* x, float* xs, long M, int C, hipStream_t st);

size_t hpe_wino4_v_floats(int B, int H, int W, int C);
int hpe_wino4_items(int B, int H, int W, int N);
hipError_t hpe_wino4_init_device();
hipError_t hpe_launch_wino4_conv3(const float* x, int lda, const float* U, const float* scale, const float* shift, float* y, int ldy, int B,
                                  int H, int W, int C, int N, int relu, float* V, hipStream_t st, int co_running, float* split_ws, int n32_below, int abl);
size_t hpe_wino4_split_ws_floats();

hipError_t hpe_launch_wino4_fused_conv3(const float* xs, const float* U, const float* scale, const float* shift, const float* zero16, float* y,
                                        int ldy, int B, int H, int W, int C, int N, int relu, hipStream_t st);
int hpe_wino4_fused_items(int B, int H, int W, int N);

hipError_t hpe_launch_gemm_bf16(GemmArgs p, int mode, int tile, hipStream_t st);
hipError_t hpe_launch_gemm_bf16_p8(GemmArgs p, int mode, hipStream_t st, int* split_k_out = nullptr);
struct ChainArgs {
    const __bf16* t2;
    const __bf16* res;
    const __bf16* x2;
    const __bf16* w2c;
    const __bf16* w2a;
    const float *scaleA, *shiftA;
    const float *scaleB, *shiftB;
    __bf16* t3;
    __bf16* u1;
    int M, ldw2c, ldw2a;
};
struct Halo3Args {
    const __bf16* x;
    const __bf16* w;
    const float* scale;
    const float* shift;
    __bf16* y;
    int M, N, ldw, relu;
    int n_ntiles;
    int two;
};
bool hpe_halo3_bf16_supported(int HW, int Cin, int N);
hipError_t hpe_launch_halo3_bf16(const Halo3Args& p, int HW, int Cin, hipStream_t st);

bool hpe_chain_bf16_supported(int C, int C4, int CP, int C2);
hipError_t hpe_launch_chain_bf16(const ChainArgs& p, int C, int C4, int CP, int C2, hipStream_t st);
hipError_t hpe_chain_bf16_occupancy(int out[3]);
struct ChainArgsF32 {
    const float *t2, *res, *w2c, *w2a, *scaleA, *shiftA, *scaleB, *shiftB;
    float *t3, *u1;
    int M, ldw2c, ldw2a, u1_slab8;
};
bool hpe_chain_f32_supported(int C, int C4, int CP);
hipError_t hpe_launch_chain_f32(const ChainArgsF32& p, int C, int C4, int CP, hipStream_t st);
hipError_t hpe_chain_f32_occupancy(int* out);
hipError_t hpe_launch_f32_to_bf16(const float* x, void* y, long n, hipStream_t st);
hipError_t hpe_launch_bf16_to_f32(const void* x, float* y, long n, hipStream_t st);
hipError_t hpe_launch_pad_input_bf16(const float* img, void* out, int B, int H, int W, int Hp, int Wp, hipStream_t st);
hipError_t hpe_launch_maxpool_bf16(const void* x, void* y, int B, int H, int C, hipStream_t st);
hipError_t hpe_launch_avgpool_bf16(const void* x, float* y, int B, int HW, int C, int ldy, hipStream_t st);

hipError_t hpe_launch_stem_fused(const float* img, const void* w, const float* scale, const float* shift, void* y, int B, int R, int bf16,
                                 hipStream_t st);
hipError_t hpe_stem_fused_init_device();
int hpe_stem_fused_pick_rows(int B);

hipError_t hpe_launch_pad_input(const float* img, float* out, int B, int H, int W, int Hp, int Wp, hipStream_t st);
hipError_t hpe_launch_maxpool(const float* x, float* y, int B, int H, int C, hipStream_t st);
hipError_t hpe_launch_avgpool(const float* x, float* y, int B, int HW, int C, int ldy, hipStream_t st);
hipError_t hpe_launch_dense_gemv(const float* x, int lda, int M, int K, const float* wt, int N, const float* scale, const float* shift, const float* res,
                                 int ldres, int relu, float* y, int ldy, hipStream_t st);
hipError_t hpe_launch_tile_theta(const float* mean85, float* theta, int B, int ld, hipStream_t st);
hipError_t hpe_launch_copy_theta(const float* src, int lds, float* dst, int ldd, int B, int n, hipStream_t st);

struct SmplDev {
    const float* v_template;
    const float* shapedirs;
    const float* posedirs;
    const float* weights;
    const float* kp_reg;
    const float* j_reg;
    const float* j_basis;
    const int* parents;
    const int* depth;
    int num_kp;
    int max_depth;
};
#define SMPL_V 6890
#define SMPL_KP_PITCH 24
#define SMPL_IMG_TILE 8
#define SMPL_SMALL_B 8

struct SmplWork {
    float* pfT;
    float* betaT;
    float* A;
    float* cams;
    float* verts_tmp;
    float* kp_part;
    int Bpad;
};

struct HpeOutputs;
hipError_t hpe_launch_smpl(const SmplDev& d, const SmplWork& w, const float* theta, int ldtheta, int B, const HpeOutputs* o,
                           hipStream_t st);
hipError_t hpe_launch_joint_regress(const float* X, const float* reg, int n, int K, float* out, const float* cams,
                                    float* kp2d, hipStream_t st);
hipError_t hpe_launch_orth_proj(const float* X, const float* cam, int B, int P, float sx, float sy, int pixels, float* out,
                                hipStream_t st);

#define SMPL_BWD_PART 512
struct SmplBwdWork {
    float* pfT;
    float* betaT;
    float* A;
    float* cams;
    float* rjg;
    float* gj;
    float* part;
    int Bpad;
};
size_t hpe_smpl_bwd_part_floats(int Bpad);
hipError_t hpe_launch_smpl_backward(const SmplDev& d, const SmplBwdWork& w, const float* theta, int B, const HpeOutputs* g,
                                    float* grad_theta, hipStream_t st);

#define CRITIC_ROWS 4
struct CriticLayerSpec {
    const char* name;
    int in, out;
};
const CriticLayerSpec* hpe_critic_layers();
struct CriticW {
    const float* w[HPE_NUM_CRITIC_DENSE];
    const float* wt[HPE_NUM_CRITIC_DENSE];
    const float* b[HPE_NUM_CRITIC_DENSE];
};
size_t hpe_critic_live_floats();
CriticW hpe_critic_live_view(const float* buf);
hipError_t hpe_launch_critic(const CriticW& w, const float* joints, int K, const float* betas, int betas_stride, const float* Rs, long N,
                             float* scores, float* kcs, hipStream_t st);
// ... 69 lines not shown
```

human-pose-estimation_amd/csrc/hpe_plan.h:

```cpp
#pragma once
#include "../../include/hpe.h"
#include "hpe_internal.h"

struct HpePlan {
    int n_streams = 2;
    int dual_gemm = 1;
    int stem_fused = 1;
    int wino_min_c = 128;
    int wino_min_items = 128;
    int wino_fused = 1;
    int wino_fused_min_hw = 28;
    int mesh_a2b = 0;
    int wino_f4 = 7;
    int wino4_fused = 0;
    int bf16_p8 = 0;
    int wino4_ksplit = 1;
    int chain_fuse = 0;
    int halo3 = 0;
    int f32_split = 0;
    int chunk_images = 0;
    int min_chunk = 32;
    int halo3_two = 4;
    int f32s_min_tiles = 128;
    int stream1x1 = 3;
    int stream1x1_min_m = 25088;
    int stream1x1_walkers = 0;
    int wino_streamk = 0;
    int concurrent_tiles = 0;
    int bf16_w8_min_tiles = 128;
    int wide128_min_tiles = 384;
    int force_wide = -1;
    int splitk_min_slabs = 4;
    int wino4_min_items = 64;
    int wino4_n32 = 256;
    int w4_abl = 0;
};

constexpr int PLAN_BF16_128_MIN_TILES = 192;
constexpr int PLAN_BF16_P8_MIN_N = 256;
constexpr int PLAN_BF16_P8_MIN_K = 512;
constexpr int PLAN_EXPAND_SMALL_GRID = 128;
constexpr int PLAN_SHORTK_TILE = TILE_128x64_W8;
constexpr int PLAN_F32S_TILE = TILE_128x128;
constexpr int PLAN_F32S_EXPAND_TILE = TILE_128x128_W8;
constexpr int PLAN_F32S_EXPAND_MIN_K = 256;

HpePlan hpe_resolve_plan(const HpeConfig& cfg);

inline int stage_bit(int hout) { return hout >= 56 ? 1 : (hout >= 28 ? 2 : (hout >= 14 ? 4 : 8)); }
inline int f4_bit(int hin) { return hin <= 7 ? 1 : (hin <= 14 ? 2 : (hin <= 28 ? 4 : 8)); }

constexpr unsigned PACK_W_SPLIT = 1u << HPE_PACK_W_SPLIT, PACK_WINO_U = 1u << HPE_PACK_WINO_U, PACK_WINO4_U = 1u << HPE_PACK_WINO4_U,
                   PACK_STEM_W = 1u << HPE_PACK_STEM_W, PACK_W_DUAL = 1u << HPE_PACK_W_DUAL, PACK_W_DUAL_SPLIT = 1u << HPE_PACK_W_DUAL_SPLIT;
unsigned layer_packs(const HpePlan& pl, bool bf16, int idx);
bool stream1x1_layer(const HpePlan& pl, bool bf16, int idx);

enum ConvKernel { CONV_K_F32 = 0, CONV_K_F32S, CONV_K_BF16, CONV_K_BF16_P8, CONV_K_HALO3, CONV_K_WINO, CONV_K_WINO_FUSED, CONV_K_WINO4, CONV_K_WINO4_FUSED };
struct ConvQuery { int B; bool concurrent, residual, workspace; };
struct ConvRoute {
    int kernel, mode, tile;
    bool in_slab8;
    bool out_slab8;
    bool concurrent;
    bool stream;
};
enum BlockJoin { JOIN_SEPARATE = 0, JOIN_DUAL, JOIN_CHAIN };
struct BlockRoute {
    ConvRoute r2a, r2b, r2c, r1;
    int join;
    bool u1_slab8;
};
struct ResBlock;
bool stream1x1_dual(const HpePlan& pl, bool bf16, const ResBlock& blk);
ConvRoute route_conv(const HpePlan& pl, bool bf16, int idx, const ConvQuery& q);
BlockRoute route_block(const HpePlan& pl, bool bf16, const ResBlock& blk, ConvQuery q);
int pick_tile(const HpePlan& pl, int M, int N, int K, bool residual_expand = false, bool concurrent = false);
int pick_tile_bf16(const HpePlan& pl, int M, int N, int K, int mode);
```

human-pose-estimation_amd/csrc/hpe_plan.hip:

```cpp
#include <hip/hip_runtime.h>

#include <climits>
#include <cmath>
#include <cstdint>
#include <cstdio>
#include <cstdlib>
#include <cstring>
#include <string>
#include <vector>

#include "gemm_contract.h"
#include "hpe_ctx.h"

namespace {

struct Network {
    std::vector<ConvSpec> specs;
    std::vector<ResBlock> blocks;
};

Network build_network() {
    Network net;
    std::vector<ConvSpec>& v = net.specs;
    auto add = [&](const std::string& n, const std::string& b, int kh, int cin, int cout, int s, int hin, int hout) {
        ConvSpec c;
        snprintf(c.name, sizeof c.name, "%s", n.c_str());
        snprintf(c.bn, sizeof c.bn, "%s", b.c_str());
        c.kh = c.kw = kh;
        c.cin = cin;
        c.cout = cout;
        c.stride = s;
        c.hin = hin;
        c.hout = hout;
        v.push_back(c);
    };
    add("conv1", "bn_conv1", 7, 3, 64, 2, 224, 112);
    const int nblk[4] = {3, 4, 6, 3};
    const int filt[4][3] = {{64, 64, 256}, {128, 128, 512}, {256, 256, 1024}, {512, 512, 2048}};
    int cin = 64, h = 56;
    int in = -1;
    for (int st = 0; st < 4; ++st) {
        for (int b = 0; b < nblk[st]; ++b) {
            const bool first = b == 0;
            const int s = (first && st > 0) ? 2 : 1;
            const int hout = h / s;
            const int i2a = (int)v.size();
            net.blocks.push_back(ResBlock{st, first, b == nblk[st] - 1, i2a, i2a + 1, i2a + 2, first ? i2a + 3 : -1, in});
            in = i2a + 2;
            char base[24], bn[24];
            snprintf(base, sizeof base, "res%d%c_branch", st + 2, 'a' + b);
            snprintf(bn, sizeof bn, "bn%d%c_branch", st + 2, 'a' + b);
            add(std::string(base) + "2a", std::string(bn) + "2a", 1, cin, filt[st][0], s, h, hout);
            add(std::string(base) + "2b", std::string(bn) + "2b", 3, filt[st][0], filt[st][1], 1, hout, hout);
            add(std::string(base) + "2c", std::string(bn) + "2c", 1, filt[st][1], filt[st][2], 1, hout, hout);
            if (first) add(std::string(base) + "1", std::string(bn) + "1", 1, cin, filt[st][2], s, h, hout);
            cin = filt[st][2];
            h = hout;
        }
    }
    return net;
}

const Network& network() {
    static const Network n = build_network();
    return n;
}

}

const std::vector<ConvSpec>& specs() { return network().specs; }
const std::vector<ResBlock>& blocks() { return network().blocks; }

struct PlanOption {
    int HpePlan::*member;
    int HpeConfig::*cfg;
    const char* env;
    int dflt[2];
    int mask[2];
    int lo, hi;
};

constexpr int ANY = -1, NO_LO = INT_MIN, NO_HI = INT_MAX;

const PlanOption kPlanOptions[] = {
    {&HpePlan::n_streams, &HpeConfig::n_streams, "HPE_STREAMS", {2, 2}, {ANY, ANY}, 1, 4},
    {&HpePlan::dual_gemm, &HpeConfig::dual_gemm, "HPE_DUAL", {1, 1}, {ANY, ANY}, NO_LO, NO_HI},
    {&HpePlan::stem_fused, &HpeConfig::stem_fused, "HPE_STEM_FUSED", {1, 1}, {ANY, ANY}, NO_LO, NO_HI},
    {&HpePlan::wino_min_c, &HpeConfig::wino_min_c, "HPE_WINO_MINC", {128, 128}, {ANY, ANY}, NO_LO, NO_HI},
    {&HpePlan::wino_min_items, &HpeConfig::wino_min_items, "HPE_WINO_MIN_ITEMS", {128, 128}, {ANY, ANY}, NO_LO, NO_HI},
    {&HpePlan::wino_fused, &HpeConfig::wino_fused, "HPE_WINO_FUSED", {1, 1}, {ANY, ANY}, NO_LO, NO_HI},
    {&HpePlan::wino_fused_min_hw, &HpeConfig::wino_fused_min_hw, "HPE_WINO_FUSED_MINHW", {28, 28}, {ANY, ANY}, NO_LO, NO_HI},
    {&HpePlan::mesh_a2b, &HpeConfig::mesh_a2b, "HPE_MESH_A2B", {0, 0}, {ANY, ANY}, NO_LO, NO_HI},
    {&HpePlan::wino_f4, &HpeConfig::wino_f4, "HPE_WINO_F4", {7, 7}, {ANY, ANY}, NO_LO, NO_HI},
    {&HpePlan::wino4_fused, &HpeConfig::wino4_fused, "HPE_WINO4_FUSED", {0, 0}, {12, 12}, NO_LO, NO_HI},
    {&HpePlan::bf16_p8, &HpeConfig::bf16_p8, "HPE_BF16_P8", {0, 0}, {ANY, ANY}, NO_LO, NO_HI},
    {&HpePlan::wino4_ksplit, &HpeConfig::wino4_ksplit, "HPE_WINO4_KSPLIT", {1, 1}, {ANY, ANY}, NO_LO, NO_HI},
    {&HpePlan::chain_fuse, &HpeConfig::chain_fuse, "HPE_CHAIN", {8, 7}, {8, 23}, NO_LO, NO_HI},
    {&HpePlan::halo3, &HpeConfig::halo3, "HPE_HALO3", {15, 15}, {0, 15}, NO_LO, NO_HI},
    {&HpePlan::f32_split, &HpeConfig::f32_split, "HPE_F32_SPLIT", {14, 14}, {15, 0}, NO_LO, NO_HI},
    {&HpePlan::chunk_images, nullptr, "HPE_CHUNK", {0, 0}, {ANY, ANY}, NO_LO, NO_HI},
    {&HpePlan::min_chunk, nullptr, "HPE_MIN_CHUNK", {32, 24}, {ANY, ANY}, NO_LO, NO_HI},
    {&HpePlan::halo3_two, nullptr, "HPE_HALO3_TWO", {4, 4}, {7, 7}, NO_LO, NO_HI},
    {&HpePlan::f32s_min_tiles, nullptr, "HPE_F32S_MIN_TILES", {128, 128}, {ANY, ANY}, NO_LO, NO_HI},
    {&HpePlan::stream1x1, nullptr, "HPE_STREAM1X1", {3, 0}, {3, 0}, 0, 3},
    {&HpePlan::stream1x1_min_m, nullptr, "HPE_STREAM1X1_MIN_M", {25088, 25088}, {ANY, ANY}, 1, NO_HI},
    {&HpePlan::stream1x1_walkers, nullptr, "HPE_STREAM1X1_WALKERS", {0, 0}, {ANY, ANY}, 0, NO_HI},
    {&HpePlan::wino_streamk, nullptr, "HPE_WINO_STREAMK", {0, 0}, {ANY, ANY}, NO_LO, NO_HI},
    {&HpePlan::concurrent_tiles, nullptr, "HPE_CONCURRENT_TILES", {0, 0}, {ANY, ANY}, NO_LO, NO_HI},
    {&HpePlan::bf16_w8_min_tiles, nullptr, "HPE_BF16_W8_MIN_TILES", {128, 128}, {ANY, ANY}, NO_LO, NO_HI},
    {&HpePlan::wide128_min_tiles, nullptr, "HPE_WIDE128_MIN_TILES", {384, 384}, {ANY, ANY}, NO_LO, NO_HI},
    {&HpePlan::force_wide, nullptr, "HPE_TILE_WIDE", {-1, -1}, {ANY, ANY}, NO_LO, NO_HI},
    {&HpePlan::splitk_min_slabs, nullptr, "HPE_SPLITK_SLABS", {4, 4}, {ANY, ANY}, 2, NO_HI},
    {&HpePlan::wino4_min_items, nullptr, "HPE_WINO4_MIN_ITEMS", {64, 64}, {ANY, ANY}, NO_LO, NO_HI},
    {&HpePlan::wino4_n32, nullptr, "HPE_WINO4_N32", {256, 256}, {ANY, ANY}, NO_LO, NO_HI},
    {&HpePlan::w4_abl, nullptr, "HPE_W4_ABL", {0, 0}, {ANY, ANY}, NO_LO, NO_HI},
};

HpePlan hpe_resolve_plan(const HpeConfig& cfg) {
    const int dt = cfg.encoder_dtype == 1 ? 1 : 0;
    HpePlan pl;
    for (const PlanOption& o : kPlanOptions) {
        int v = o.dflt[dt];
        const char* e = getenv(o.env);
        if (o.cfg && cfg.*o.cfg >= 0) v = cfg.*o.cfg;
        else if (e && o.member == &HpePlan::mesh_a2b) v = e[0] == 'v' ? 1 : (e[0] == 'm' ? 2 : 0);
        else if (e) v = atoi(e);
        v &= o.mask[dt];
        pl.*o.member = v < o.lo ? o.lo : (v > o.hi ? o.hi : v);
    }
    if (pl.min_chunk < 8) pl.min_chunk = dt ? 24 : 32;
    pl.wino_fused = pl.wino_fused && pl.wino_min_c > 0;
    if (pl.wino_min_c <= 0) pl.wino_f4 = pl.wino4_fused = 0;
    return pl;
}

static int pick_f32s(const HpePlan& pl, bool split_packed, int M, int N, int K, bool residual_expand) {
    if (!split_packed || N <= 64) return -1;
    if (residual_expand && K < PLAN_F32S_EXPAND_MIN_K) return -1;
    const int tile = residual_expand ? PLAN_F32S_EXPAND_TILE : PLAN_F32S_TILE;
    const TileShape ts = tile_shape(GEMM_K_F32S, tile);
    return (long)((M + ts.bm - 1) / ts.bm) * ((N + ts.bn - 1) / ts.bn) >= pl.f32s_min_tiles ? tile : -1;
}

int pick_tile(const HpePlan& pl, int M, int N, int K, bool residual_expand, bool concurrent) {
    const bool wide = N > 64;
    if (wide && residual_expand) return (long)((M + 127) / 128) * ((N + 63) / 64) < PLAN_EXPAND_SMALL_GRID ? TILE_64x64 : TILE_128x64_W8;
    if (wide && pl.force_wide >= 0) return pl.force_wide;
    if (!wide) return TILE_128x64;
    if (K <= 128 && M >= 150000) return PLAN_SHORTK_TILE;
    if ((concurrent || pl.concurrent_tiles) && pl.wide128_min_tiles > 0 && (long)((M + 127) / 128) * ((N + 127) / 128) >= pl.wide128_min_tiles) return TILE_128x128;
    if (M >= 150000) return TILE_64x128;
    return TILE_64x64;
}

static int pick_bf16(const HpePlan& pl, int M, int N, int K, bool residual_expand, bool concurrent, int mode) {
    if (pl.bf16_p8 && N >= PLAN_BF16_P8_MIN_N && N % 256 == 0 && K >= PLAN_BF16_P8_MIN_K && !residual_expand) {
        const int bit = mode == GEMM_CONV3 ? (N == 256 ? 1 : 2) : (mode == GEMM_DUAL ? (N >= 2048 ? 8 : 16) : 4);
        if (pl.bf16_p8 & bit) return TILE_P8_256x256;
    }
    if (N <= 64) return TILE_128x64;
    const long t128 = (long)((M + 127) / 128) * ((N + 127) / 128);
    int tile = t128 >= ((concurrent || pl.concurrent_tiles) ? PLAN_BF16_128_MIN_TILES : 512) ? TILE_128x128 : TILE_64x128;
    if (residual_expand) tile = TILE_128x64_W8;
    else if (M <= 16384 && M >= 8192 && K >= 1024 && N >= 256) tile = TILE_256x128_W8;
    if (pl.bf16_w8_min_tiles > 0 && t128 >= pl.bf16_w8_min_tiles) tile = TILE_128x128_W8;
    return tile;
}

int pick_tile_bf16(const HpePlan& pl, int M, int N, int K, int mode) { return pick_bf16(pl, M, N, K, false, false, mode); }

unsigned layer_packs(const HpePlan& pl, bool bf16, int idx) {
    const ConvSpec& s = specs()[idx];
    unsigned m = idx == 0 ? PACK_STEM_W : 0;
    const int slab = bf16 ? 64 : 32;
    const ResBlock* blk = nullptr;
    for (const ResBlock& b : blocks())
        if (b.first && b.i2c == idx) blk = &b;
    if (pl.dual_gemm && blk && s.cin % slab == 0 && specs()[blk->i1].cin % slab == 0) {
        m |= PACK_W_DUAL;
        if (!bf16 && (pl.f32_split & stage_bit(s.hout))) m |= PACK_W_DUAL_SPLIT;
    }
    if (bf16) return m;
    if (idx != 0 && s.kh == 1 && (pl.f32_split & stage_bit(s.hout))) m |= PACK_W_SPLIT;
    const bool wino = s.kh == 3 && s.stride == 1 && s.cin % 32 == 0 && s.cout % 64 == 0;
    if (wino && pl.wino_min_c > 0 && (s.cin >= pl.wino_min_c || (pl.wino_fused && s.hin >= pl.wino_fused_min_hw))) m |= PACK_WINO_U;
    if (wino && ((pl.wino_f4 | pl.wino4_fused) & f4_bit(s.hin))) m |= PACK_WINO4_U;
    return m;
}

static bool use_chain(const HpePlan& pl, bool bf16, const ResBlock& blk);
bool stream1x1_layer(const HpePlan& pl, bool bf16, int idx) {
    if (bf16 || !(pl.stream1x1 & 1) || !pl.f32_split) return false;
    const ConvSpec& s = specs()[idx];
    for (const ResBlock& b : blocks())
        if (b.i2c == idx && !b.first && !use_chain(pl, bf16, b))
            return s.kh == 1 && s.stride == 1 && s.cout == 4 * s.cin && hpe_stream_f32s_supported(1, s.cout, conv_k_pad(idx, bf16));
    return false;
}

bool stream1x1_dual(const HpePlan& pl, bool bf16, const ResBlock& blk) {
    if (bf16 || !(pl.stream1x1 & 2) || !pl.f32_split || !blk.first || use_chain(pl, bf16, blk) || !(layer_packs(pl, bf16, blk.i2c) & PACK_W_DUAL)) return false;
    const ConvSpec& s2 = specs()[blk.i2c];
    const ConvSpec& s1 = specs()[blk.i1];
    return hpe_stream_f32s_dual_supported(1, s2.cout, s2.cin, s1.cin, s1.stride, s1.hin, s1.hout);
}

static ConvRoute route_gemm(const HpePlan& pl, bool bf16, int mode, int M, int N, int K, bool expand, bool split_packed, bool concurrent,
                            bool stream_layer = false) {
    ConvRoute r{CONV_K_F32, mode, -1, false, false, concurrent, stream_layer && expand && M >= pl.stream1x1_min_m};
    if (bf16) {
        r.tile = pick_bf16(pl, M, N, K, expand, concurrent, mode);
        r.kernel = r.tile == TILE_P8_256x256 ? CONV_K_BF16_P8 : CONV_K_BF16;
    } else if ((r.tile = pick_f32s(pl, split_packed, M, N, K, expand)) >= 0) {
        r.kernel = CONV_K_F32S;
    } else {
        r.tile = pick_tile(pl, M, N, K, expand, concurrent);
    }
    return r;
}

ConvRoute route_conv(const HpePlan& pl, bool bf16, int idx, const ConvQuery& q) {
    const ConvSpec& s = specs()[idx];
    const unsigned packs = layer_packs(pl, bf16, idx);
    const int B = q.B, H = s.hin;
    const int mode = idx == 0 ? GEMM_STEM : s.kh == 3 ? GEMM_CONV3 : s.stride == 1 ? GEMM_DENSE : GEMM_STRIDED;
    const bool plain3 = mode == GEMM_CONV3 && s.stride == 1 && !q.residual;
    auto special = [&](int kernel) { return ConvRoute{kernel, mode, -1, kernel == CONV_K_WINO_FUSED || kernel == CONV_K_WINO4_FUSED, false, q.concurrent}; };
    const int min4 = pl.wino_min_items < pl.wino4_min_items ? pl.wino_min_items : pl.wino4_min_items;
    if (plain3 && (packs & PACK_WINO4_U) && (pl.wino4_fused & f4_bit(H)) && hpe_wino4_fused_items(B, H, H, s.cout) >= min4) return special(CONV_K_WINO4_FUSED);
    const bool f4 = plain3 && (packs & PACK_WINO4_U) && (pl.wino_f4 & f4_bit(H)) && hpe_wino4_items(B, H, H, s.cout) >= min4;
    if (plain3 && !f4 && pl.wino_fused && (packs & PACK_WINO_U) && H >= pl.wino_fused_min_hw && hpe_wino_fused_items(B, H, H, s.cout) >= pl.wino_min_items)
        return special(CONV_K_WINO_FUSED);
    if (f4 && q.workspace) return special(CONV_K_WINO4);
    if (plain3 && (packs & PACK_WINO_U) && q.workspace && s.cin >= pl.wino_min_c &&
        (long)((B * ((H + 1) / 2) * ((H + 1) / 2) + 63) / 64) * (s.cout / 64) >= pl.wino_min_items)
        return special(CONV_K_WINO);
    if (bf16 && plain3 && (pl.halo3 & f4_bit(H)) && hpe_halo3_bf16_supported(H, s.cin, s.cout)) return special(CONV_K_HALO3);
    return route_gemm(pl, bf16, mode, B * s.hout * s.hout, s.cout, conv_k_pad(idx, bf16), mode == GEMM_DENSE && q.residual && s.cout == 4 * s.cin,
                      (packs & PACK_W_SPLIT) != 0, q.concurrent, stream1x1_layer(pl, bf16, idx));
}

static bool use_chain(const HpePlan& pl, bool bf16, const ResBlock& blk) {
    if (blk.last) return false;
    const int stg = blk.stage, i2c = blk.i2c;
    const ConvSpec& s2 = specs()[i2c];
    const ConvSpec& sn = specs()[i2c + (blk.first ? 2 : 1)];
    if (sn.kh != 1 || sn.stride != 1 || sn.cin != s2.cout) return false;
    if (!bf16) return !blk.first && stg == 0 && (pl.chain_fuse & 8) && hpe_chain_f32_supported(s2.cin, s2.cout, sn.cout);
    if (blk.first) {
        const ConvSpec& s1 = specs()[blk.i1];
        return stg == 0 && (pl.chain_fuse & 4) && (layer_packs(pl, bf16, i2c) & PACK_W_DUAL) && s1.stride == 1 && s1.hin == s2.hin &&
               hpe_chain_bf16_supported(s2.cin, s2.cout, sn.cout, s1.cin);
    }
    const int bit = stg == 0 ? 1 : stg == 1 ? 2 : stg == 2 ? 16 : 0;
    return (pl.chain_fuse & bit) && hpe_chain_bf16_supported(s2.cin, s2.cout, sn.cout, 0);
}

BlockRoute route_block(const HpePlan& pl, bool bf16, const ResBlock& blk, ConvQuery q) {
    BlockRoute b{};
    q.residual = false;
    b.r2a = route_conv(pl, bf16, blk.i2a, q);
    b.r2b = route_conv(pl, bf16, blk.i2b, q);
    b.r2a.out_slab8 = b.r2b.in_slab8;
    const ConvSpec& s2 = specs()[blk.i2c];
    if (use_chain(pl, bf16, blk)) {
        b.join = JOIN_CHAIN;
        b.u1_slab8 = route_conv(pl, bf16, blk.i2c + (blk.first ? 3 : 2), q).in_slab8;
    } else if (blk.first && (layer_packs(pl, bf16, blk.i2c) & PACK_W_DUAL)) {
        b.join = JOIN_DUAL;
        b.r2c = route_gemm(pl, bf16, GEMM_DUAL, q.B * s2.hout * s2.hout, s2.cout, s2.cin + specs()[blk.i1].cin, false,
                           (layer_packs(pl, bf16, blk.i2c) & PACK_W_DUAL_SPLIT) != 0, q.concurrent);
        b.r2c.stream = stream1x1_dual(pl, bf16, blk) && q.B * s2.hout * s2.hout >= pl.stream1x1_min_m;
    } else {
        if (blk.first) b.r1 = route_conv(pl, bf16, blk.i1, q);
        q.residual = true;
        b.r2c = route_conv(pl, bf16, blk.i2c, q);
    }
    return b;
}
```

human-pose-estimation_amd/engine.py:

```python
from __future__ import annotations

import ctypes as C

import numpy as np

from . import _lib
from .critic_spec import PARAM_FLOATS
from .regressor_spec import PARAM_FLOATS as REGRESSOR_PARAM_FLOATS
from .resnet_spec import CONV_SPECS, ENCODER_PARAM_FLOATS, ENCODER_STAT_FLOATS

NUM_VERTS = _lib.NUM_VERTS


def _torch():
    import torch

    return torch


def _require_cuda_tensor(t, name, shape_tail=None):
    torch = _torch()
    if not isinstance(t, torch.Tensor):
        raise TypeError("%s must be a torch.Tensor on the GPU" % name)
    if not t.is_cuda:
# ... 775 lines not shown
            x, dy = self._bf16_arg(x, "x"), self._bf16_arg(dy, "dy")
            dx = self._new_bf16(*x.shape)
            _lib.check(self.lib.hpe_debug_maxpool_backward_mixed(x.data_ptr(), dy.data_ptr(), x.shape[0], x.shape[1], x.shape[3], dx.data_ptr(),
                                                                 self._stream()))
            return dx
        x, dy = _require_cuda_tensor(x, "x"), _require_cuda_tensor(dy, "dy")
        dx = self._new(*x.shape)
        _lib.check(self.lib.hpe_debug_maxpool_backward(x.data_ptr(), dy.data_ptr(), x.shape[0], x.shape[1], x.shape[3], dx.data_ptr(), self._stream()))
        return dx

    def debug_avgpool_backward(self, dy, HW, precision="fp32"):
        dy = _require_cuda_tensor(dy, "dy")
        if self._mixed(precision):
            dx = self._new_bf16(dy.shape[0], HW, dy.shape[1])
            _lib.check(self.lib.hpe_debug_avgpool_backward_mixed(dy.data_ptr(), dy.shape[0], HW, dy.shape[1], dx.data_ptr(), self._stream()))
            return dx
        dx = self._new(dy.shape[0], HW, dy.shape[1])
        _lib.check(self.lib.hpe_debug_avgpool_backward(dy.data_ptr(), dy.shape[0], HW, dy.shape[1], dx.data_ptr(), self._stream()))
        return dx

    def encoder_stash(self, idx, precision="fp32"):
        if self._mixed(precision):
            B = self.lib.hpe_debug_encoder_stash_batch_mixed(self._h)
            if B < 1:
                raise _lib.HpeError("encoder_stash: no mixed-precision training forward has run")
            s = CONV_SPECS[idx] if idx >= 0 else None
            out = self._new_bf16(B, s.hout, s.hout, s.cout) if s else self._new_bf16(B, 56, 56, 64)
            _lib.check(self.lib.hpe_debug_encoder_stash_mixed(self._h, idx, out.data_ptr(), self._stream()))
            return out
        B = self.lib.hpe_debug_encoder_stash_batch(self._h)
        if B < 1:
            raise _lib.HpeError("encoder_stash: no training forward has run")
        s = CONV_SPECS[idx] if idx >= 0 else None
        out = self._new(B, s.hout, s.hout, s.cout) if s else self._new(B, 56, 56, 64)
        _lib.check(self.lib.hpe_debug_encoder_stash(self._h, idx, out.data_ptr(), self._stream()))
        return out

    def mesh_loss(self, seg, verts2d):
        torch = _torch()
        seg = _require_cuda_tensor(seg, "seg")
        verts2d = _require_cuda_tensor(verts2d, "verts2d")
        B, H, W = seg.shape[0], seg.shape[1], seg.shape[2]
        P = verts2d.shape[1]
        out = torch.zeros(4, dtype=torch.float32, device=self.tdev)
        _lib.check(self.lib.hpe_mesh_loss(self._h, seg.data_ptr(), verts2d.data_ptr(), B, H, W, P, out.data_ptr(), self._stream()))
        return out[0]

    def mesh_loss_grad(self, seg, verts2d, want_neighbours=False):
        torch = _torch()
        seg = _require_cuda_tensor(seg, "seg")
        verts2d = _require_cuda_tensor(verts2d, "verts2d")
        if seg.dim() != 3 or verts2d.dim() != 3 or verts2d.shape[2] != 2 or verts2d.shape[0] != seg.shape[0]:
            raise ValueError("seg must be [B,H,W] and verts2d [B,P,2], got %s and %s" % (tuple(seg.shape), tuple(verts2d.shape)))
        B, H, W = seg.shape[0], seg.shape[1], seg.shape[2]
        P = verts2d.shape[1]
        out = torch.zeros(4, dtype=torch.float32, device=self.tdev)
        grad = torch.empty((B, P, 2), dtype=torch.float32, device=self.tdev)
        nn_pix = nn_vert = None
        if want_neighbours:
            nn_pix = torch.empty((B, H, W), dtype=torch.int32, device=self.tdev)
            nn_vert = torch.empty((B, P), dtype=torch.int32, device=self.tdev)
        _lib.check(self.lib.hpe_mesh_loss_grad(self._h, seg.data_ptr(), verts2d.data_ptr(), B, H, W, P, out.data_ptr(), grad.data_ptr(),
                                               nn_pix.data_ptr() if want_neighbours else None,
                                               nn_vert.data_ptr() if want_neighbours else None, self._stream()))
        return (out[0], grad, nn_pix, nn_vert) if want_neighbours else (out[0], grad)

    def val_losses(self, kp_gt, kp2d_stages, seg=None, verts2d_stages=None, out=None):
        torch = _torch()
        kp_gt = _require_cuda_tensor(kp_gt, "kp_gt")
        n = len(kp2d_stages)
        kp2d = [_require_cuda_tensor(t, "kp2d") for t in kp2d_stages]
        B, K = kp_gt.shape[0], kp_gt.shape[1]
        kp_ptrs = (C.c_void_p * n)(*[t.data_ptr() for t in kp2d])
        H = W = P = 0
        seg_ptr, v_ptrs, keep = None, None, None
        if seg is not None and verts2d_stages is not None:
            seg = _require_cuda_tensor(seg, "seg")
            keep = [_require_cuda_tensor(t, "verts2d") for t in verts2d_stages]
            if len(keep) != n or seg.shape[0] != B:
                raise ValueError("one verts2d tensor per stage and one silhouette per image are needed")
            H, W, P = seg.shape[1], seg.shape[2], keep[0].shape[1]
            seg_ptr = seg.data_ptr()
            v_ptrs = (C.c_void_p * n)(*[t.data_ptr() for t in keep])
        if out is None:
            out = torch.empty((n, 4), dtype=torch.float32, device=self.tdev)
        _lib.check(self.lib.hpe_val_losses(self._h, seg_ptr, kp_gt.data_ptr(), kp_ptrs, v_ptrs, n, B, K, H, W, P, out.data_ptr(), self._stream()))
        return out

    def check_device(self):
        _lib.check(self.lib.hpe_device_status(self._h, self._stream()))

    def debug_conv(self, idx, x, residual=None, relu=True):
        s = CONV_SPECS[idx]
        x = _require_cuda_tensor(x, "x")
        B = x.shape[0]
        y = self._new(B, s.hout, s.hout, s.cout)
        r = None
        if residual is not None:
            r = _require_cuda_tensor(residual, "residual").data_ptr()
        _lib.check(self.lib.hpe_debug_conv(self._h, idx, x.data_ptr(), B, r, int(relu), y.data_ptr(), self._stream()))
        return y

    def conv_route(self, idx, B, concurrent=False, residual=False, workspace=True):
        return _lib.conv_route(self.lib, self._cfg, idx, B, concurrent, residual, workspace)

    def debug_dual(self, idx2c, t2, x):
        s = CONV_SPECS[idx2c]
        t2 = _require_cuda_tensor(t2, "t2")
        x = _require_cuda_tensor(x, "x")
        B = t2.shape[0]
        y = self._new(B, s.hout, s.hout, s.cout)
        _lib.check(self.lib.hpe_debug_dual(self._h, int(idx2c), t2.data_ptr(), x.data_ptr(), B, y.data_ptr(), self._stream()))
        return y

    def conv_stream1x1(self, idx, B, concurrent=False, residual=True):
        return int(self.lib.hpe_debug_conv_stream1x1(C.byref(self._cfg), int(idx), int(B), int(concurrent), int(residual)))

    def _debug_gemm(self, call, what, mode, tile, x, wt, y, M, N, K, kw):
        g = _lib.HpeDebugGemm()
        g.struct_size = C.sizeof(_lib.HpeDebugGemm)
        fields = dict(lda=K, ldw=K, ldy=N, ldres=N, mode=mode, tile=tile, x=x, wt=wt, y=y, M=M, N=N, K=K)
        fields.update(kw)
        for k, v in fields.items():
            if k in ("x", "x2", "wt", "residual", "scale", "shift", "y"):
                v = v.data_ptr() if hasattr(v, "data_ptr") else v
            elif k in ("struct_size", "split_k") or not hasattr(g, k):
                raise TypeError("%s: unknown argument %r" % (what, k))
            setattr(g, k, v)
        sk = C.c_int(-1)
        g.split_k = C.pointer(sk)
        _lib.check(call(g))
        return sk.value

    def debug_gemm_ex(self, mode, tile, x, wt, y, M, N, K, **kw):
        return self._debug_gemm(lambda g: self.lib.hpe_debug_gemm_ex(self._h, C.byref(g), self._stream()), "debug_gemm_ex", mode, tile, x, wt, y, M, N, K, kw)

    def debug_gemm_launch(self, kernel, mode, tile, x, wt, y, M, N, K, w_piece=0, **kw):
        return self._debug_gemm(lambda g: self.lib.hpe_debug_gemm_launch(self._h, C.byref(g), int(kernel), int(w_piece), self._stream()),
                                "debug_gemm_launch", mode, tile, x, wt, y, M, N, K, kw)

    def debug_chain(self, idx2c, t2, residual):
        s = CONV_SPECS[idx2c]
        first = CONV_SPECS[idx2c + 1].name.endswith("branch1")
        sn = CONV_SPECS[idx2c + (2 if first else 1)]
        t2 = _require_cuda_tensor(t2, "t2", (s.hin, s.hin, s.cin))
        residual = _require_cuda_tensor(residual, "residual", (s.hout, s.hout, CONV_SPECS[idx2c + 1].cin if first else s.cout))
        B = t2.shape[0]
        t3 = self._new(B, s.hout, s.hout, s.cout)
        u1 = self._new(B, sn.hout, sn.hout, sn.cout)
        occ = (C.c_int * 3)()
        _lib.check(self.lib.hpe_debug_chain(self._h, idx2c, t2.data_ptr(), residual.data_ptr(), B, t3.data_ptr(), u1.data_ptr(), occ, self._stream()))
        return t3, u1, (occ[0], occ[1], occ[2])

    def debug_stem(self, images, rows_per_strip=0):
        images = _require_cuda_tensor(images, "images", (224, 224, 3))
        y = self._new(images.shape[0], 56, 56, 64)
        _lib.check(self.lib.hpe_debug_stem(self._h, images.data_ptr(), images.shape[0], int(rows_per_strip), y.data_ptr(), self._stream()))
        return y

    def joint_regress(self, X, use_kp_regressor=True):
        X = _require_cuda_tensor(X, "X", (NUM_VERTS, 3))
        K = self.num_kp if use_kp_regressor else 24
        out = self._new(X.shape[0], K, 3)
        _lib.check(self.lib.hpe_debug_joint_regress(self._h, X.data_ptr(), X.shape[0], int(use_kp_regressor), out.data_ptr(), self._stream()))
        return out

    def encoder_kernel_description(self):
        if self.encoder_dtype == "fp32":
            return ("conv_gemm_f32s_dma_kernel (the 1x1 / strided / dual-source layers of stages 3-5 on the bf16 matrix cores, operands split "
                    "exactly into three bf16 pieces) + conv_gemm_f32_dma_kernel (the other 1x1 layers) + w4_input_kernel + w4_gemm_kernel / w4_gemm32_kernel "
                    "(the 13 3x3 layers on the 28x28 / 14x14 / 7x7 maps as fp32 Winograd F(4x4,3x3); F(2x2,3x3) / direct below 64 work "
                    "items) + wino_fused_split_kernel (the three 56x56 3x3 layers, F(2x2,3x3) on the bf16 matrix cores through the same exact split) + stem_fused_f32s_kernel (image and weights split like the 1x1 layers) -- the 53 conv layers of one "
                    "step, priced at their direct-convolution FLOPs")
        return ("conv_gemm_bf16_dma_kernel (1x1 / strided / dual-source layers) + chain_expand_reduce_bf16_kernel (branch2c + next branch2a of "
                "stages 2-3 as one launch) + conv3_halo_bf16_kernel (the sixteen 3x3 layers, tile + halo resident in LDS) + stem_fused_bf16_kernel "
                "-- the 53 conv layers of one step, priced at their algorithmic HBM bytes")

    def enable_timing(self, level=1):
        _lib.check(self.lib.hpe_enable_timing(self._h, int(level)))

    def timings(self):
        ms = (C.c_float * 5)()
        _lib.check(self.lib.hpe_get_timings(self._h, ms))
        return dict(encoder_ms=ms[0], conv_ms=ms[1], regress_smpl_ms=ms[2], total_ms=ms[4])

    def span_stats(self):
        ms = (C.c_float * 3)()
        n = C.c_int()
        _lib.check(self.lib.hpe_get_span_stats(self._h, ms, C.byref(n)))
        return dict(mean_ms=ms[0], min_ms=ms[1], max_ms=ms[2], calls=n.value)

    def set_loss_counter(self, counter=None):
        _lib.check(self.lib.hpe_debug_set_loss_counter(self._h, None if counter is None else counter.data_ptr()))
        self._loss_counter = counter

    def loss_timings(self):
        ms = (C.c_float * 2)()
        _lib.check(self.lib.hpe_get_loss_timings(self._h, ms))
        return dict(val_losses_ms=ms[0], a2b_search_ms=ms[1])

    def conv_timings(self):
        ms = (C.c_float * _lib.NUM_CONV)()
        _lib.check(self.lib.hpe_get_conv_timings(self._h, ms))
        return list(ms)


def _cur_stream(t):
    return C.c_void_p(_torch().cuda.current_stream(t.device).cuda_stream)


def orth_proj(X, camera):
    X = _require_cuda_tensor(X, "X")
    camera = _require_cuda_tensor(camera, "camera").reshape(-1, 3)
    B, P = X.shape[0], X.shape[1]
    out = _torch().empty((B, P, 2), dtype=_torch().float32, device=X.device)
    with _torch().cuda.device(X.device):
        _lib.check(_lib.load().hpe_orth_proj(X.data_ptr(), camera.data_ptr(), B, P, out.data_ptr(), _cur_stream(X)))
    return out


def reproject(verts, cam, im_w, im_h):
    verts = _require_cuda_tensor(verts, "verts")
    cam = _require_cuda_tensor(cam, "cam").reshape(-1, 3)
    B, P = verts.shape[0], verts.shape[1]
    out = _torch().empty((B, P, 2), dtype=_torch().float32, device=verts.device)
    with _torch().cuda.device(verts.device):
        _lib.check(
            _lib.load().hpe_reproject_vertices(verts.data_ptr(), cam.data_ptr(), B, P, float(im_w), float(im_h), out.data_ptr(), _cur_stream(verts))
        )
    return out


def kp_loss_backward(kp_gt, kp_pred, grad_loss=None):
    kp_gt = _require_cuda_tensor(kp_gt, "kp_gt")
    kp_pred = _require_cuda_tensor(kp_pred, "kp_pred")
    B, K = kp_gt.shape[0], kp_gt.shape[1]
    gl = None
    if grad_loss is not None:
        grad_loss = _require_cuda_tensor(grad_loss.reshape(1), "grad_loss")
        gl = grad_loss.data_ptr()
    out = _torch().empty((B, K, 2), dtype=_torch().float32, device=kp_gt.device)
    with _torch().cuda.device(kp_gt.device):
        _lib.check(_lib.load().hpe_kp_loss_backward(kp_gt.data_ptr(), kp_pred.data_ptr(), B, K, gl, out.data_ptr(), _cur_stream(kp_gt)))
    return out


def kp_loss_parts(kp_gt, kp_pred):
    kp_gt = _require_cuda_tensor(kp_gt, "kp_gt")
    kp_pred = _require_cuda_tensor(kp_pred, "kp_pred")
    B, K = kp_gt.shape[0], kp_gt.shape[1]
    out = _torch().zeros(4, dtype=_torch().float32, device=kp_gt.device)
    with _torch().cuda.device(kp_gt.device):
        _lib.check(_lib.load().hpe_kp_loss(kp_gt.data_ptr(), kp_pred.data_ptr(), B, K, out.data_ptr(), _cur_stream(kp_gt)))
    return out[:3]
```

include/hpe.h:

```cpp
#ifndef HPE_H_
#define HPE_H_

#ifdef __cplusplus
extern "C" {
#endif

#define HPE_OK 0
#define HPE_ERR_INVALID 1
#define HPE_ERR_HIP 2
#define HPE_ERR_STATE 3
#define HPE_ERR_NO_DEVICE 4
#define HPE_ERR_REDUCE 5

#define HPE_NUM_CONV 53
#define HPE_NUM_DENSE 3
#define HPE_NUM_CRITIC_DENSE 9
#define HPE_NUM_VERTS 6890
#define HPE_NUM_JOINTS 24
#define HPE_NUM_BETAS 10
#define HPE_NUM_POSE_BASIS 207
#define HPE_THETA_DIM 85
#define HPE_FEATURE_DIM 2048
#define HPE_MAX_KP 24
#define HPE_IMG_SIZE 224
// ... 253 lines not shown
    int idct_group0;
    int store_group0;
    unsigned char quant[3][64];
} HpeJpegImage;

int hpe_jpeg_info(int B, const unsigned char* const* streams, const long long* lengths, HpeJpegInfo* info_out);
int hpe_jpeg_decode(int B, const unsigned char* const* streams, const long long* lengths, const int* channels, int threads,
                    short* coef_out, long long coef_capacity, HpeJpegImage* table_out, int* status_out, long long* totals_out);
int hpe_jpeg_backend(const HpeJpegImage* table_host, const HpeJpegImage* table_dev, int B, const short* coef_dev, long long coef_count,
                     unsigned char* workspace_dev, long long workspace_bytes, unsigned char* frames_dev, long long frames_bytes,
                     void* stream);

#define HPE_JPEG_ENC_HEADER_BYTES 640
#define HPE_JPEG_ENC_BLOCK_BYTES 416
typedef struct HpeJpegEncImage {
    long long frame_offset;
    long long coef_offset[3];
    int H, W;
    int C;
    int hmax, vmax;
    int blocks_w[3], blocks_h[3];
    int real_w[3], real_h[3];
    int group0;
    unsigned char quant[2][64];
} HpeJpegEncImage;

int hpe_jpeg_encode_layout(int B, const int* shapes, const long long* frame_offsets, int hmax, int vmax, int quality,
                           HpeJpegEncImage* table_out, long long* totals_out);
int hpe_jpeg_forward(const HpeJpegEncImage* table_host, const HpeJpegEncImage* table_dev, int B, const unsigned char* frames_dev,
                     long long frames_bytes, short* coef_dev, long long coef_count, void* stream);
int hpe_jpeg_entropy_encode(const HpeJpegEncImage* table, int B, const short* coef, long long coef_count, int units, int xdensity,
                            int ydensity, int threads, unsigned char* out, long long out_capacity, long long* offsets_out,
                            long long* lengths_out);

#define HPE_PNG_MAX_SIDE 16384
#define HPE_PNG_STORE_BYTES_PER_GROUP 1024
typedef struct HpePngImage {
    long long raw_offset;
    long long pal_offset;
    long long work_offset;
    long long out_offset;
    int H, W;
    int color_type;
    int depth;
    int channels;
    int rowbytes;
    int bpp;
    int store_group0;
} HpePngImage;

int hpe_png_backend(const HpePngImage* table_host, const HpePngImage* table_dev, int B, const unsigned char* raw_dev, long long raw_bytes,
                    unsigned char* workspace_dev, long long workspace_bytes, unsigned char* frames_dev, long long frames_bytes,
                    void* stream);

typedef struct HpePngFilterImage {
    long long frame_offset;
    long long scan_offset;
    int H, W;
    int C;
    int row0;
} HpePngFilterImage;

int hpe_png_filter(const HpePngFilterImage* table_host, const HpePngFilterImage* table_dev, int B, const unsigned char* frames_dev,
                   long long frames_bytes, unsigned char* scan_dev, long long scan_bytes, void* stream);

#define HPE_DRAW_JOINTS 19
#define HPE_DRAW_MAX_RADIUS 256
int hpe_draw_panels(const float* images, const float* kp_gt, const float* kp_pred, const unsigned char* rend_img,
                    const unsigned char* rend_seg, const int* skeleton, int n, int T, int S, unsigned char* out, void* stream);
int hpe_draw_skeleton(unsigned char* images, const float* joints, const unsigned char* vis, const int* skeleton, int n, int H, int W,
                      int draw_edges, int radius, void* stream);

typedef struct hpe_renderer hpe_renderer;

typedef struct HpeRenderParams {
    int struct_size;
    int color_id;
    int do_alpha;
    int rot_axis;
    float rot_deg;
    float near;
    float far;
} HpeRenderParams;

void hpe_render_params_init(HpeRenderParams* p);
int hpe_renderer_create(int device, const int* faces_host, int Fn, int P, int max_batch, hpe_renderer** out);
int hpe_renderer_destroy(hpe_renderer* r);
int hpe_render(hpe_renderer* r, const float* verts_dev, const float* cam_dev, int B, int H, int W, const unsigned char* bg_dev,
               const HpeRenderParams* p, unsigned char* out_dev, void* stream);

int hpe_debug_render_ids(hpe_renderer* r, const float* verts_dev, const float* cam_dev, int B, int H, int W, const HpeRenderParams* p,
                         int* face_dev, float* z_dev, void* stream);
int hpe_debug_render_vertices(hpe_renderer* r, const float* verts_dev, const float* cam_dev, int B, int H, int W, const HpeRenderParams* p,
                              void* rec_dev, void* stream);

int hpe_debug_conv(hpe_ctx* ctx, int idx, const float* x_dev, int B, const float* residual_dev, int relu, float* y_dev,
                   void* stream);
int hpe_debug_chain(hpe_ctx* ctx, int idx2c, const float* t2_dev, const float* residual_dev, int B, float* t3_dev, float* u1_dev,
                    int* occupancy, void* stream);
int hpe_debug_stem(hpe_ctx* ctx, const float* images_dev, int B, int rows_per_strip, float* y_dev, void* stream);
#define HPE_GEMM_DENSE 0
#define HPE_GEMM_STRIDED 1
#define HPE_GEMM_CONV3 2
#define HPE_GEMM_DUAL 4
typedef struct HpeDebugGemm {
    int struct_size;
    int mode;
    int tile;
    int M, N, K;
    int lda, ldw, ldy, ldres, w_rows;
    int relu;
    int Hi, Wi, Cin, Ho, Wo, stride;
    int k1_slabs;
    int y_slab8;
    int use_splitk;
    int reserved;
    const float* x;
    const float* x2;
    const float* wt;
    const float* residual;
    const float* scale;
    const float* shift;
    float* y;
    int* split_k;
} HpeDebugGemm;
int hpe_debug_gemm_ex(hpe_ctx* ctx, const HpeDebugGemm* g, void* stream);
int hpe_debug_gemm_check(const HpeDebugGemm* g, int kernel, int w_piece);
int hpe_debug_gemm_launch(hpe_ctx* ctx, const HpeDebugGemm* g, int kernel, int w_piece, void* stream);
enum {
    HPE_CONV_K_F32 = 0,
    HPE_CONV_K_F32S,
    HPE_CONV_K_BF16,
    HPE_CONV_K_BF16_P8,
    HPE_CONV_K_HALO3,
    HPE_CONV_K_WINO,
    HPE_CONV_K_WINO_FUSED,
    HPE_CONV_K_WINO4,
    HPE_CONV_K_WINO4_FUSED,
    HPE_CONV_K_COUNT
};
typedef struct HpeConvRoute {
    int struct_size;
    int kernel;
    int mode;
    int tile;
    int in_slab8, out_slab8;
    int join, join_kernel, join_tile, next_slab8;
    unsigned packs;
    int reserved;
} HpeConvRoute;
int hpe_debug_conv_route(const HpeConfig* cfg, int idx, int B, int concurrent, int residual, int workspace, HpeConvRoute* out);
int hpe_debug_conv_stream1x1(const HpeConfig* cfg, int idx, int B, int concurrent, int residual);
int hpe_debug_dual(hpe_ctx* ctx, int idx2c, const float* t2_dev, const float* x_dev, int B, float* y_dev, void* stream);
int hpe_debug_gemm(hpe_ctx* ctx, const float* x_dev, const float* wt_dev, int M, int N, int K, int w_rows, int tile,
                   const float* residual_dev, int relu, float* y_dev, void* stream);
int hpe_debug_maxpool(const float* x_dev, int B, int H, int C, float* y_dev, void* stream);
int hpe_debug_avgpool(const float* x_dev, int B, int HW, int C, float* y_dev, void* stream);
int hpe_debug_joint_regress(hpe_ctx* ctx, const float* X_dev, int n, int use_kp_regressor, float* out_dev, void* stream);
int hpe_enable_timing(hpe_ctx* ctx, int level);
int hpe_device_status(hpe_ctx* ctx, void* stream);
int hpe_get_timings(hpe_ctx* ctx, float ms[5]);
int hpe_get_span_stats(hpe_ctx* ctx, float ms[3], int* n_calls);
int hpe_get_loss_timings(hpe_ctx* ctx, float ms[2]);
int hpe_debug_set_loss_counter(hpe_ctx* ctx, void* counter_dev);
int hpe_get_conv_timings(hpe_ctx* ctx, float* ms53);

#ifdef __cplusplus
}
#endif
#endif
```

Baseline: 23000 images/sec.

## Add persistent fp32-split streaming chain kernel fusing branch2c with next block's 2a

Adds a persistent walker kernel for the stage-2 residual blocks that computes branch2c (with residual add or dual-source projection) using three-piece bf16 split MFMAs, writes t3, and then feeds the result straight into the next block's 1x1 branch2a reduction in registers and LDS to produce u1. It is enabled by default through stream1x1 bits 4 and 8, and takes over from the existing chain or dual join for the large-M blocks. The aim is to avoid a separate launch and the re-read of the 256-channel output, and to overlap loads through double-buffered LDS DMA. In exchange the kernel uses a lot of LDS and registers, which limits occupancy, and accumulating the split partial sums across waves adds some overhead.

Measured after the change: 23550 images/sec (median of 6 runs). 1.02x the previous value.

```diff
diff --git a/human-pose-estimation_amd/_lib.py b/human-pose-estimation_amd/_lib.py
--- a/human-pose-estimation_amd/_lib.py
+++ b/human-pose-estimation_amd/_lib.py
@@ -298,6 +298,7 @@
     "hpe_debug_conv_route": (C.c_int, [C.POINTER(HpeConfig), C.c_int, C.c_int, C.c_int, C.c_int, C.c_int, C.POINTER(HpeConvRoute)]),
     "hpe_debug_conv_stream1x1": (C.c_int, [C.POINTER(HpeConfig), C.c_int, C.c_int, C.c_int, C.c_int]),
     "hpe_debug_dual": (C.c_int, [C.c_void_p, C.c_int, C.c_void_p, C.c_void_p, C.c_int, C.c_void_p, C.c_void_p]),
+    "hpe_debug_stream_chain": (C.c_int, [C.c_void_p, C.c_int, C.c_void_p, C.c_void_p, C.c_int, C.c_void_p, C.c_void_p, C.c_int, C.c_int, C.c_void_p]),
     "hpe_debug_maxpool": (C.c_int, [C.c_void_p, C.c_int, C.c_int, C.c_int, C.c_void_p, C.c_void_p]),
     "hpe_debug_avgpool": (C.c_int, [C.c_void_p, C.c_int, C.c_int, C.c_int, C.c_void_p, C.c_void_p]),
     "hpe_debug_joint_regress": (C.c_int, [C.c_void_p, C.c_void_p, C.c_int, C.c_int, C.c_void_p, C.c_void_p]),
diff --git a/human-pose-estimation_amd/build.py b/human-pose-estimation_amd/build.py
--- a/human-pose-estimation_amd/build.py
+++ b/human-pose-estimation_amd/build.py
@@ -9,7 +9,7 @@
 CSRC = os.path.join(HERE, "csrc")
 LIBDIR = os.path.join(HERE, "lib")
 LIB = os.path.join(LIBDIR, "libhpe_hip.so")
-SOURCES = ["conv_gemm.hip", "conv_gemm_f32s.hip", "conv_stream_f32s.hip", "conv_gemm_bf16.hip", "conv_gemm_bf16_p8.hip", "conv_chain_bf16.hip", "conv_chain_f32.hip", "conv3_halo_bf16.hip", "conv_wino.hip", "conv_wino4.hip", "stem_fused.hip", "encoder_ops.hip", "smpl.hip", "losses.hip", "prepost.hip", "render.hip", "hpe_plan.hip", "hpe_finalize.hip", "hpe_encoder.hip", "hpe_api.hip", "hpe_render_api.hip", "smpl_bwd.hip", "critic.hip", "critic_train.hip", "regressor_train.hip", "augment.hip", "encoder_train.hip", "encoder_grad.hip", "encoder_grad_bf16.hip", "encoder_repack.hip", "encoder_bn.hip", "jpeg_entropy.hip", "jpeg_decode.hip", "jpeg_huffman_enc.hip", "jpeg_encode.hip", "png_decode.hip", "png_encode.hip", "draw.hip", "adam.hip", "eval_scores.hip"]
+SOURCES = ["conv_gemm.hip", "conv_gemm_f32s.hip", "conv_stream_f32s.hip", "conv_stream_chain_f32s.hip", "conv_gemm_bf16.hip", "conv_gemm_bf16_p8.hip", "conv_chain_bf16.hip", "conv_chain_f32.hip", "conv3_halo_bf16.hip", "conv_wino.hip", "conv_wino4.hip", "stem_fused.hip", "encoder_ops.hip", "smpl.hip", "losses.hip", "prepost.hip", "render.hip", "hpe_plan.hip", "hpe_finalize.hip", "hpe_encoder.hip", "hpe_api.hip", "hpe_render_api.hip", "smpl_bwd.hip", "critic.hip", "critic_train.hip", "regressor_train.hip", "augment.hip", "encoder_train.hip", "encoder_grad.hip", "encoder_grad_bf16.hip", "encoder_repack.hip", "encoder_bn.hip", "jpeg_entropy.hip", "jpeg_decode.hip", "jpeg_huffman_enc.hip", "jpeg_encode.hip", "png_decode.hip", "png_encode.hip", "draw.hip", "adam.hip", "eval_scores.hip"]
 CFLAGS = ["--offload-arch=gfx950", "-O3", "-std=c++17", "-fPIC", "-fvisibility=hidden", "-fno-fast-math"]
 
 
diff --git a/human-pose-estimation_amd/csrc/conv_stream_chain_f32s.hip b/human-pose-estimation_amd/csrc/conv_stream_chain_f32s.hip
--- /dev/null
+++ b/human-pose-estimation_amd/csrc/conv_stream_chain_f32s.hip
@@ -0,0 +1,240 @@
+#include <hip/hip_runtime.h>
+#include <stdint.h>
+
+#include "bf16_split.h"
+#include "conv_gemm_common.h"
+#include "hpe_internal.h"
+#include "lds_dma.h"
+
+namespace {
+
+constexpr int CBM = 32, CNW = 8, CN4 = 256, CNP = 64;
+
+constexpr int chain_k(int s, int hi, int t) { return 16 * s + 8 * (t >> 2) + 4 * hi + (t & 3); }
+
+__device__ __forceinline__ void split8(const f32x4& lo, const f32x4& up, bf16x8& h0, bf16x8& h1, bf16x8& h2) {
+    bf16_split3_cast<8>([&](int e) { return e < 4 ? lo[e] : up[e - 4]; }, h0, h1, h2);
+}
+
+__device__ __forceinline__ void six(const bf16x8 (&w)[3], const bf16x8& b0, const bf16x8& b1, const bf16x8& b2, f32x16& acc, f32x16& x) {
+    x = __builtin_amdgcn_mfma_f32_32x32x16_bf16(w[0], b2, x, 0, 0, 0);
+    x = __builtin_amdgcn_mfma_f32_32x32x16_bf16(w[1], b1, x, 0, 0, 0);
+    x = __builtin_amdgcn_mfma_f32_32x32x16_bf16(w[2], b0, x, 0, 0, 0);
+    x = __builtin_amdgcn_mfma_f32_32x32x16_bf16(w[0], b1, x, 0, 0, 0);
+    x = __builtin_amdgcn_mfma_f32_32x32x16_bf16(w[1], b0, x, 0, 0, 0);
+    acc = __builtin_amdgcn_mfma_f32_32x32x16_bf16(w[0], b0, acc, 0, 0, 0);
+}
+
+template <int K, bool DUAL>
+__global__ __launch_bounds__(64 * CNW, 2) void conv_stream_chain_f32s_kernel(StreamChainArgs p, int walkers) {
+    constexpr int NRES = DUAL ? 0 : 4;
+    constexpr int NST = 4;
+    constexpr int KS = K / 16;
+    constexpr int CH = K / 8;
+    constexpr int RAW_BYTES = CBM * K * 4;
+    constexpr int PLANE_BYTES = CBM * K * 2;
+    constexpr int PART_BYTES = CBM * CNP * 4;
+    constexpr int STAGE_BYTES = CBM * CN4 * 4;
+    constexpr int AP = RAW_BYTES / 1024 / CNW;
+    constexpr int UNITS = CBM * CH;
+    static_assert((K == 64 && !DUAL) || (K == 128 && DUAL), "identity chain: K = 64; conv_block chain: K = 64 + 64");
+    static_assert(AP >= 1 && UNITS <= 64 * CNW && UNITS % 64 == 0, "tile geometry");
+
+    __shared__ __attribute__((aligned(16))) float lds[(3 * PLANE_BYTES + CNW * PART_BYTES + STAGE_BYTES) / 4 + 2 * CNP];
+    __shared__ __attribute__((aligned(16))) float raw_lds[2 * RAW_BYTES / 4];
+    char* const work = reinterpret_cast<char*>(lds);
+    char* const part = work + 3 * PLANE_BYTES;
+    char* const raw = reinterpret_cast<char*>(raw_lds);
+    char* const stage = part + CNW * PART_BYTES;
+    float* const bnB = reinterpret_cast<float*>(stage + STAGE_BYTES);
+
+    const int walker = blockIdx.x;
+    const int n_mtiles = p.M / CBM;
+    if (walker >= walkers || walker >= n_mtiles) return;
+    const int cnt = (n_mtiles - walker + walkers - 1) / walkers;
+
+    const int t = threadIdx.x;
+    const int lane = t & 63;
+    const int wave = __builtin_amdgcn_readfirstlane(t >> 6);
+    const int hi = lane >> 5;
+    const int px = lane & 31;
+
+    bf16x8 wexp[KS][3], wred[2][2][3];
+    {
+        const float* wa = p.wA + (size_t)(32 * wave + px) * p.ldwA + 8 * hi;
+#pragma unroll
+        for (int q = 0; q < KS; ++q) {
+            split8(*reinterpret_cast<const f32x4*>(wa + 16 * q), *reinterpret_cast<const f32x4*>(wa + 16 * q + 4), wexp[q][0], wexp[q][1], wexp[q][2]);
+            if (q % 4 == 3) asm volatile("" ::: "memory");
+        }
+#pragma unroll
+        for (int nb = 0; nb < 2; ++nb)
+#pragma unroll
+            for (int s = 0; s < 2; ++s) {
+                const float* wb = p.wB + (size_t)(32 * nb + px) * p.ldwB + 32 * wave + chain_k(s, hi, 0);
+                static_assert(chain_k(0, 0, 4) - chain_k(0, 0, 0) == 8 && chain_k(1, 1, 0) == 20, "two runs of 4, 8 apart");
+                split8(*reinterpret_cast<const f32x4*>(wb), *reinterpret_cast<const f32x4*>(wb + 8), wred[nb][s][0], wred[nb][s][1], wred[nb][s][2]);
+            }
+    }
+
+    unsigned dma_off[AP];
+#pragma unroll
+    for (int i = 0; i < AP; ++i) {
+        const int s = (CNW * i + wave) * 64 + lane;
+        dma_off[i] = (unsigned)(s / (K / 4)) * 64 + ((s % (K / 4)) * 4 & 63);
+    }
+    const float *src_t2 = p.t2, *src_x = p.x;
+    asm volatile("" : "+s"(src_t2), "+s"(src_x));
+    const float* const dma_src = (DUAL && (lane & 16)) ? src_x : src_t2;
+    const int sp_r = (t % UNITS) / CH, sp_c = t % CH;
+    const int sp_src = sp_r * (K * 4) + sp_c * 32;
+    const int sp_dst = sp_r * (K * 2) + ((sp_c ^ ((sp_r / (16 / CH)) & (CH - 1))) << 4);
+    const int a_row = px * (K * 2);
+    const int a_x = (px / (16 / CH)) & (CH - 1);
+    const unsigned t3_off = (unsigned)px * CN4 + 32 * wave + 4 * hi;
+    const int ur = p.u1_slab8 ? (t & 31) : (t >> 4);
+    const int uc = p.u1_slab8 ? (((t >> 6) << 1) | ((t >> 5) & 1)) : (t & 15);
+    const char* const part_r = part + ur * 256 + ((uc ^ (ur & 15)) << 4);
+    const unsigned u1_off = p.u1_slab8 ? ((unsigned)(uc >> 1) * p.M + ur) * 8 + (uc & 1) * 4 : (unsigned)ur * CNP + uc * 4;
+    const unsigned u1_tile = p.u1_slab8 ? CBM * 8 : CBM * CNP;
+    if (t < CNP) bnB[t] = p.scaleB[t], bnB[CNP + t] = p.shiftB[t];
+    cfloat_p scp = (cfloat_p)(p.scaleA + 32 * wave);
+    cfloat_p shp = (cfloat_p)(p.shiftA + 32 * wave);
+
+    auto issue_tile = [&](int m0, int buf, f32x4 (&rnext)[4]) {
+        asm volatile("" ::: "memory");
+#pragma unroll
+        for (int i = 0; i < AP; ++i) {
+            dma16(dma_src + (size_t)m0 * 64 + dma_off[i], raw + buf * RAW_BYTES + (CNW * i + wave) * 1024);
+        }
+        asm volatile("" ::: "memory");
+#pragma unroll
+        for (int j = 0; j < NRES; ++j) rnext[j] = HPE_RES_LOAD(reinterpret_cast<const f32x4*>(p.x + (size_t)m0 * CN4 + (t3_off + 8 * j)));
+        asm volatile("" ::: "memory");
+    };
+
+    auto tile_step = [&](int k, int buf, f32x4 (&rcur)[4], f32x4 (&rnext)[4]) {
+        const int m0 = (walker + k * walkers) * CBM;
+        const int m0n = k + 1 < cnt ? m0 + walkers * CBM : m0;
+        wait_counts<NRES + NST + 1>();
+        bare_barrier();
+        if (t < UNITS) {
+            const unsigned rb = (unsigned)(uintptr_t)(const __attribute__((address_space(3))) char*)(raw + buf * RAW_BYTES);
+            f32x4 lo, up;
+            asm volatile("ds_read_b128 %0, %2\n\tds_read_b128 %1, %2 offset:16\n\ts_waitcnt lgkmcnt(0)" : "=&v"(lo), "=&v"(up) : "v"(rb + sp_src) : "memory");
+            bf16x8 h0, h1, h2;
+            split8(lo, up, h0, h1, h2);
+            *reinterpret_cast<bf16x8*>(work + sp_dst) = h0;
+            *reinterpret_cast<bf16x8*>(work + PLANE_BYTES + sp_dst) = h1;
+            *reinterpret_cast<bf16x8*>(work + 2 * PLANE_BYTES + sp_dst) = h2;
+        }
+        lds_barrier();
+        issue_tile(m0n, buf ^ 1, rnext);
+
+        f32x16 acc, acx;
+#pragma unroll
+        for (int e = 0; e < 16; ++e) acc[e] = acx[e] = 0.f;
+        bf16x8 b[2][3];
+        auto read_b = [&](int q, bf16x8 (&d)[3]) {
+            const int off = a_row + (((2 * q + hi) ^ a_x) << 4);
+#pragma unroll
+            for (int pc = 0; pc < 3; ++pc) d[pc] = *reinterpret_cast<const bf16x8*>(work + pc * PLANE_BYTES + off);
+        };
+        read_b(0, b[0]);
+#pragma unroll
+        for (int q = 0; q < KS; ++q) {
+            if (q + 1 < KS) read_b(q + 1, b[(q + 1) & 1]);
+            asm volatile("" ::: "memory");
+            six(wexp[q], b[q & 1][0], b[q & 1][1], b[q & 1][2], acc, acx);
+        }
+        acc += acx;
+        if (!DUAL) wait_counts<AP + NRES + NST + 1>();
+        cfloat_p scq = scp, shq = shp;
+        asm volatile("" : "+s"(scq), "+s"(shq));
+        int pxq = px;
+        if (DUAL) asm volatile("" : "+v"(pxq));
+        char* const stage_w = stage + pxq * 1024;
+        char* const part_w = part + wave * PART_BYTES + pxq * 256;
+        bf16x8 tb[2][3];
+        float* const t3p = p.t3 + (size_t)m0 * CN4;
+#pragma unroll
+        for (int s = 0; s < 2; ++s) {
+            f32x4 o[2];
+#pragma unroll
+            for (int jj = 0; jj < 2; ++jj) {
+                const int j = 2 * s + jj;
+                const f32x4 sc_lo = *reinterpret_cast<cf32x4_p>(scq + 8 * j), sc_hi = *reinterpret_cast<cf32x4_p>(scq + 8 * j + 4);
+                const f32x4 sh_lo = *reinterpret_cast<cf32x4_p>(shq + 8 * j), sh_hi = *reinterpret_cast<cf32x4_p>(shq + 8 * j + 4);
+#pragma unroll
+                for (int i = 0; i < 4; ++i) {
+                    float v = acc[4 * j + i] * (hi ? sc_hi[i] : sc_lo[i]) + (hi ? sh_hi[i] : sh_lo[i]);
+                    if (!DUAL) v += rcur[j][i];
+                    o[jj][i] = fmaxf(v, 0.f);
+                }
+                *reinterpret_cast<f32x4*>(stage_w + (((8 * wave + 2 * j + hi) ^ (px & 15)) << 4)) = o[jj];
+            }
+            split8(o[0], o[1], tb[s][0], tb[s][1], tb[s][2]);
+        }
+#pragma unroll
+        for (int nb = 0; nb < 2; ++nb) {
+            f32x16 r, rx;
+#pragma unroll
+            for (int e = 0; e < 16; ++e) r[e] = rx[e] = 0.f;
+#pragma unroll
+            for (int s = 0; s < 2; ++s) six(wred[nb][s], tb[s][0], tb[s][1], tb[s][2], r, rx);
+            r += rx;
+#pragma unroll
+            for (int j = 0; j < 4; ++j) {
+                f32x4 v;
+#pragma unroll
+                for (int i = 0; i < 4; ++i) v[i] = r[4 * j + i];
+                *reinterpret_cast<f32x4*>(part_w + (((8 * nb + 2 * j + hi) ^ (px & 15)) << 4)) = v;
+            }
+        }
+        wait_counts<AP + NRES + NST + 1, 0>();
+        bare_barrier();
+#pragma unroll
+        for (int i = 0; i < NST; ++i) {
+            const int r = 8 * i + wave;
+            const f32x4 v = *reinterpret_cast<const f32x4*>(stage + r * 1024 + ((lane ^ (r & 15)) << 4));
+            __builtin_nontemporal_store(v, reinterpret_cast<f32x4*>(t3p + (r * CN4 + 4 * lane)));
+        }
+        f32x4 u = *reinterpret_cast<const f32x4*>(part_r);
+#pragma unroll
+        for (int w = 1; w < CNW; ++w) u += *reinterpret_cast<const f32x4*>(part_r + w * PART_BYTES);
+        const f32x4 scB = *reinterpret_cast<const f32x4*>(bnB + 4 * uc), shB = *reinterpret_cast<const f32x4*>(bnB + CNP + 4 * uc);
+#pragma unroll
+        for (int i = 0; i < 4; ++i) u[i] = fmaxf(u[i] * scB[i] + shB[i], 0.f);
+        *reinterpret_cast<f32x4*>(p.u1 + (size_t)(m0 / CBM) * u1_tile + u1_off) = u;
+    };
+
+    f32x4 ra[4], rb[4];
+    issue_tile(walker * CBM, 0, ra);
+    wait_counts<0>();
+    for (int k = 0; k < cnt; k += 2) {
+        tile_step(k, 0, ra, rb);
+        if (k + 1 < cnt) tile_step(k + 1, 1, rb, ra);
+    }
+    wait_counts<0>();
+}
+
+}
+
+bool hpe_stream_chain_f32s_supported(int M, int C, int C4, int CP, int C2) {
+    return M > 0 && M % CBM == 0 && C == 64 && C4 == CN4 && CP == CNP && (C2 == 0 || C2 == 64);
+}
+
+hipError_t hpe_launch_stream_chain_f32s(const StreamChainArgs& p, int C, int C4, int CP, int C2, int max_walkers, hipStream_t st) {
+    if (!hpe_stream_chain_f32s_supported(p.M, C, C4, CP, C2)) return hipErrorInvalidValue;
+    if (!p.t2 || !p.x || !p.wA || !p.wB || !p.t3 || !p.u1 || !p.scaleA || !p.shiftA || !p.scaleB || !p.shiftB) return hipErrorInvalidValue;
+    if (p.ldwA < C + C2 || p.ldwB < C4 || (p.ldwA % 4) != 0 || (p.ldwB % 4) != 0) return hipErrorInvalidValue;
+    if ((((uintptr_t)p.t2 | (uintptr_t)p.x | (uintptr_t)p.wA | (uintptr_t)p.wB | (uintptr_t)p.t3 | (uintptr_t)p.u1 | (uintptr_t)p.scaleA | (uintptr_t)p.shiftA |
+          (uintptr_t)p.scaleB | (uintptr_t)p.shiftB) & 15) != 0)
+        return hipErrorInvalidValue;
+    int walkers = hpe_stream_device_cus();
+    if (max_walkers > 0 && walkers > max_walkers) walkers = max_walkers;
+    if (walkers > p.M / CBM) walkers = p.M / CBM;
+    if (C2) hipLaunchKernelGGL((conv_stream_chain_f32s_kernel<128, true>), dim3(walkers), dim3(64 * CNW), 0, st, p, walkers);
+    else hipLaunchKernelGGL((conv_stream_chain_f32s_kernel<64, false>), dim3(walkers), dim3(64 * CNW), 0, st, p, walkers);
+    return hipGetLastError();
+}
diff --git a/human-pose-estimation_amd/csrc/conv_stream_f32s.hip b/human-pose-estimation_amd/csrc/conv_stream_f32s.hip
--- a/human-pose-estimation_amd/csrc/conv_stream_f32s.hip
+++ b/human-pose-estimation_amd/csrc/conv_stream_f32s.hip
@@ -148,7 +148,9 @@
     wait_counts<0>();
 }
 
-int device_cus() {
+}
+
+int hpe_stream_device_cus() {
     static int n = 0;
     if (n == 0) {
         int dev = 0, v = 0;
@@ -156,8 +158,6 @@
         else n = 256;
     }
     return n;
-}
-
 }
 
 bool hpe_stream_f32s_supported(int M, int N, int K) { return M > 0 && (K == 64 || K == 128) && N >= SBN && N % SBN == 0; }
@@ -175,7 +175,7 @@
     p.n_ntiles = p.N / SBN;
     p.split_k = 1;
     p.res_prefetch = 1;
-    int walkers = 2 * device_cus() / p.n_ntiles;
+    int walkers = 2 * hpe_stream_device_cus() / p.n_ntiles;
     if (max_walkers > 0 && walkers > max_walkers) walkers = max_walkers;
     if (walkers > p.n_mtiles) walkers = p.n_mtiles;
     if (walkers < 1) walkers = 1;
diff --git a/human-pose-estimation_amd/csrc/hpe_api.hip b/human-pose-estimation_amd/csrc/hpe_api.hip
--- a/human-pose-estimation_amd/csrc/hpe_api.hip
+++ b/human-pose-estimation_amd/csrc/hpe_api.hip
@@ -831,6 +831,22 @@
     return fail(HPE_ERR_INVALID, "hpe_debug_dual: idx2c must be the branch2c of a conv_block that this plan runs as the dual-source launch");
 }
 
+int hpe_debug_stream_chain(hpe_ctx* c, int idx2c, const float* t2, const float* x, int B, float* t3, float* u1, int slab8, int rows, void* stream) {
+    int rc = check_ready(c, B, NEED_ENC);
+    if (rc) return rc;
+    if (!t2 || !x || !t3 || !u1 || c->bf16 || rows < 0) return fail(HPE_ERR_INVALID, "hpe_debug_stream_chain: null pointer, negative rows, or a bf16 context");
+    for (const ResBlock& blk : blocks()) {
+        if (blk.i2c != idx2c || blk.last) continue;
+        const ConvSpec& s2 = specs()[blk.i2c];
+        const ConvSpec& sn = specs()[blk.i2c + (blk.first ? 2 : 1)];
+        if (rows > B * s2.hout * s2.hout || sn.cin != s2.cout || (blk.first && specs()[blk.i1].stride != 1)) break;
+        DeviceGuard g(c->cfg.device);
+        if (run_stream_chain(c, blk.i2c, blk.first, t2, x, B, t3, u1, static_cast<hipStream_t>(stream), slab8 != 0, rows) != hipSuccess) break;
+        return HPE_OK;
+    }
+    return fail(HPE_ERR_INVALID, "hpe_debug_stream_chain: refused (idx2c must be res2a_branch2c or res2b_branch2c, rows a multiple of 32 inside the batch); nothing was launched");
+}
+
 int hpe_debug_gemm(hpe_ctx* c, const float* x, const float* wt, int M, int N, int K, int w_rows, int tile, const float* residual,
                    int relu, float* y, void* stream) {
     if (!c || !c->finalized || !c->have_regressor) return fail(HPE_ERR_STATE, "needs a finalized ctx with the regressor loaded");
diff --git a/human-pose-estimation_amd/csrc/hpe_ctx.h b/human-pose-estimation_amd/csrc/hpe_ctx.h
--- a/human-pose-estimation_amd/csrc/hpe_ctx.h
+++ b/human-pose-estimation_amd/csrc/hpe_ctx.h
@@ -305,6 +305,8 @@
                          const float* scale = nullptr, const float* shift = nullptr);
 hipError_t run_chain(hpe_ctx* c, int i2c, bool first, const float* t2, const float* res, int B, float* t3, float* u1, hipStream_t st,
                      bool u1_slab8 = false);
+hipError_t run_stream_chain(hpe_ctx* c, int i2c, bool first, const float* t2, const float* x, int B, float* t3, float* u1, hipStream_t st,
+                            bool u1_slab8, int rows = 0);
 hipError_t encoder_impl(hpe_ctx* c, const float* images, int B, float* features, int ldfeat, hipStream_t st);
 hipError_t run_dense(hpe_ctx* c, const float* x, int lda, int M, int K, const float* w, int w_rows, int N, const float* scale, const float* shift,
                      const float* res, int ldres, int relu, float* y, int ldy, hipStream_t st, float* partial = nullptr, size_t partial_floats = 0);
diff --git a/human-pose-estimation_amd/csrc/hpe_encoder.hip b/human-pose-estimation_amd/csrc/hpe_encoder.hip
--- a/human-pose-estimation_amd/csrc/hpe_encoder.hip
+++ b/human-pose-estimation_amd/csrc/hpe_encoder.hip
@@ -155,6 +155,24 @@
     p.M = B * s2.hout * s2.hout;
     p.ldw2a = Ln.k_pad;
     return hpe_launch_chain_bf16(p, s2.cin, s2.cout, sn.cout, first ? specs()[i2c + 1].cin : 0, st);
+}
+
+hipError_t run_stream_chain(hpe_ctx* c, int i2c, bool first, const float* t2, const float* x, int B, float* t3, float* u1, hipStream_t st,
+                            bool u1_slab8, int rows) {
+    const ConvSpec& s2 = specs()[i2c];
+    const int inext = i2c + (first ? 2 : 1);
+    const ConvSpec& sn = specs()[inext];
+    const ConvLayer& L2 = c->conv[i2c];
+    const ConvLayer& Ln = c->conv[inext];
+    if (c->bf16 || (first && (!L2.w_dual || !L2.shift_dual))) return hipErrorInvalidValue;
+    StreamChainArgs q{};
+    q.t2 = t2, q.x = x, q.t3 = t3, q.u1 = u1;
+    q.wA = first ? L2.w_dual : L2.w, q.ldwA = first ? L2.k_dual : L2.k_pad;
+    q.scaleA = first ? c->ones : L2.scale, q.shiftA = first ? L2.shift_dual : L2.shift;
+    q.wB = Ln.w, q.ldwB = Ln.k_pad, q.scaleB = Ln.scale, q.shiftB = Ln.shift;
+    q.M = rows ? rows : B * s2.hout * s2.hout;
+    q.u1_slab8 = u1_slab8 ? 1 : 0;
+    return hpe_launch_stream_chain_f32s(q, s2.cin, s2.cout, sn.cout, first ? specs()[i2c + 1].cin : 0, c->plan.stream1x1_walkers, st);
 }
 
 hipError_t run_dense(hpe_ctx* c, const float* x, int lda, int M, int K, const float* w, int w_rows, int N, const float* scale,
@@ -239,7 +257,19 @@
         have_2a = false;
         HIPE(timed_conv(c, i2b, br.r2b, T1, B, nullptr, 1, T2, st, wv, slot));
         const float* res = cur;
-        if (br.join == JOIN_CHAIN) {
+        if (br.stream_chain) {
+            const bool t2 = c->timing >= 2;
+            if (t2) HIPE(hipEventRecord(c->cev0[i2c], st));
+            HIPE(run_stream_chain(c, i2c, first, T2, cur, B, nxt, T1, st, br.stream_u1_slab8));
+            if (t2) {
+                HIPE(hipEventRecord(c->cev1[i2c], st));
+                if (first) {
+                    HIPE(hipEventRecord(c->cev0[i1], st));
+                    HIPE(hipEventRecord(c->cev1[i1], st));
+                }
+            }
+            have_2a = true;
+        } else if (br.join == JOIN_CHAIN) {
             const bool t2 = c->timing >= 2;
             if (t2) HIPE(hipEventRecord(c->cev0[i2c], st));
             HIPE(run_chain(c, i2c, first, T2, cur, B, nxt, T1, st, br.u1_slab8));
diff --git a/human-pose-estimation_amd/csrc/hpe_internal.h b/human-pose-estimation_amd/csrc/hpe_internal.h
--- a/human-pose-estimation_amd/csrc/hpe_internal.h
+++ b/human-pose-estimation_amd/csrc/hpe_internal.h
@@ -49,6 +49,14 @@
 bool hpe_stream_f32s_supported(int M, int N, int K);
 bool hpe_stream_f32s_dual_supported(int M, int N, int K1, int K2, int stride, int Hi, int Ho);
 hipError_t hpe_launch_stream_f32s(GemmArgs p, int mode, int max_walkers, hipStream_t st);
+int hpe_stream_device_cus();
+struct StreamChainArgs {
+    const float *t2, *x, *wA, *wB, *scaleA, *shiftA, *scaleB, *shiftB;
+    float *t3, *u1;
+    int M, ldwA, ldwB, u1_slab8;
+};
+bool hpe_stream_chain_f32s_supported(int M, int C, int C4, int CP, int C2);
+hipError_t hpe_launch_stream_chain_f32s(const StreamChainArgs& p, int C, int C4, int CP, int C2, int max_walkers, hipStream_t st);
 
 size_t hpe_wino_v_floats(int B, int H, int W, int C);
 hipError_t hpe_wino_init_device();
diff --git a/human-pose-estimation_amd/csrc/hpe_plan.h b/human-pose-estimation_amd/csrc/hpe_plan.h
--- a/human-pose-estimation_amd/csrc/hpe_plan.h
+++ b/human-pose-estimation_amd/csrc/hpe_plan.h
@@ -22,7 +22,7 @@
     int min_chunk = 32;
     int halo3_two = 4;
     int f32s_min_tiles = 128;
-    int stream1x1 = 3;
+    int stream1x1 = 15;
     int stream1x1_min_m = 25088;
     int stream1x1_walkers = 0;
     int wino_streamk = 0;
@@ -69,6 +69,8 @@
     ConvRoute r2a, r2b, r2c, r1;
     int join;
     bool u1_slab8;
+    bool stream_chain;
+    bool stream_u1_slab8;
 };
 struct ResBlock;
 bool stream1x1_dual(const HpePlan& pl, bool bf16, const ResBlock& blk);
diff --git a/human-pose-estimation_amd/csrc/hpe_plan.hip b/human-pose-estimation_amd/csrc/hpe_plan.hip
--- a/human-pose-estimation_amd/csrc/hpe_plan.hip
+++ b/human-pose-estimation_amd/csrc/hpe_plan.hip
@@ -102,7 +102,7 @@
     {&HpePlan::min_chunk, nullptr, "HPE_MIN_CHUNK", {32, 24}, {ANY, ANY}, NO_LO, NO_HI},
     {&HpePlan::halo3_two, nullptr, "HPE_HALO3_TWO", {4, 4}, {7, 7}, NO_LO, NO_HI},
     {&HpePlan::f32s_min_tiles, nullptr, "HPE_F32S_MIN_TILES", {128, 128}, {ANY, ANY}, NO_LO, NO_HI},
-    {&HpePlan::stream1x1, nullptr, "HPE_STREAM1X1", {3, 0}, {3, 0}, 0, 3},
+    {&HpePlan::stream1x1, nullptr, "HPE_STREAM1X1", {15, 0}, {15, 0}, 0, 15},
     {&HpePlan::stream1x1_min_m, nullptr, "HPE_STREAM1X1_MIN_M", {25088, 25088}, {ANY, ANY}, 1, NO_HI},
     {&HpePlan::stream1x1_walkers, nullptr, "HPE_STREAM1X1_WALKERS", {0, 0}, {ANY, ANY}, 0, NO_HI},
     {&HpePlan::wino_streamk, nullptr, "HPE_WINO_STREAMK", {0, 0}, {ANY, ANY}, NO_LO, NO_HI},
@@ -256,6 +256,16 @@
     return (pl.chain_fuse & bit) && hpe_chain_bf16_supported(s2.cin, s2.cout, sn.cout, 0);
 }
 
+static bool stream_chain(const HpePlan& pl, bool bf16, const ResBlock& blk, int join, int M) {
+    if (bf16 || !pl.f32_split || blk.last || M < pl.stream1x1_min_m) return false;
+    if (!(pl.stream1x1 & (join == JOIN_CHAIN ? 4 : join == JOIN_DUAL ? 8 : 0))) return false;
+    const ConvSpec& s2 = specs()[blk.i2c];
+    const ConvSpec& sn = specs()[blk.i2c + (blk.first ? 2 : 1)];
+    if (sn.kh != 1 || sn.stride != 1 || sn.cin != s2.cout || s2.hout != s2.hin) return false;
+    if (blk.first && (specs()[blk.i1].stride != 1 || specs()[blk.i1].hin != s2.hin)) return false;
+    return hpe_stream_chain_f32s_supported(M, s2.cin, s2.cout, sn.cout, blk.first ? specs()[blk.i1].cin : 0);
+}
+
 BlockRoute route_block(const HpePlan& pl, bool bf16, const ResBlock& blk, ConvQuery q) {
     BlockRoute b{};
     q.residual = false;
@@ -276,5 +286,7 @@
         q.residual = true;
         b.r2c = route_conv(pl, bf16, blk.i2c, q);
     }
+    b.stream_chain = stream_chain(pl, bf16, blk, b.join, q.B * s2.hout * s2.hout);
+    if (b.stream_chain) b.stream_u1_slab8 = route_conv(pl, bf16, blk.i2c + (blk.first ? 3 : 2), q).in_slab8;
     return b;
 }
diff --git a/human-pose-estimation_amd/engine.py b/human-pose-estimation_amd/engine.py
--- a/human-pose-estimation_amd/engine.py
+++ b/human-pose-estimation_amd/engine.py
@@ -951,6 +951,23 @@
         _lib.check(self.lib.hpe_debug_chain(self._h, idx2c, t2.data_ptr(), residual.data_ptr(), B, t3.data_ptr(), u1.data_ptr(), occ, self._stream()))
         return t3, u1, (occ[0], occ[1], occ[2])
 
+    def debug_stream_chain(self, idx2c, t2, x, slab8=False, rows=0):
+        s = CONV_SPECS[idx2c]
+        first = CONV_SPECS[idx2c + 1].name.endswith("branch1")
+        sn = CONV_SPECS[idx2c + (2 if first else 1)]
+        t2 = _require_cuda_tensor(t2, "t2", (s.hin, s.hin, s.cin))
+        x = _require_cuda_tensor(x, "x", (s.hout, s.hout, CONV_SPECS[idx2c + 1].cin if first else s.cout))
+        B = t2.shape[0]
+        t3 = self._new(B, s.hout, s.hout, s.cout)
+        M = int(rows) if rows else B * sn.hout * sn.hout
+        u1 = self._new(sn.cout // 8, M, 8) if slab8 else self._new(B, sn.hout, sn.hout, sn.cout)
+        if rows:
+            t3.zero_()
+            u1.zero_()
+        _lib.check(self.lib.hpe_debug_stream_chain(self._h, int(idx2c), t2.data_ptr(), x.data_ptr(), B, t3.data_ptr(), u1.data_ptr(), int(bool(slab8)),
+                                                   int(rows), self._stream()))
+        return t3, u1
+
     def debug_stem(self, images, rows_per_strip=0):
         images = _require_cuda_tensor(images, "images", (224, 224, 3))
         y = self._new(images.shape[0], 56, 56, 64)
diff --git a/include/hpe.h b/include/hpe.h
--- a/include/hpe.h
+++ b/include/hpe.h
@@ -429,6 +429,8 @@
 int hpe_debug_conv_route(const HpeConfig* cfg, int idx, int B, int concurrent, int residual, int workspace, HpeConvRoute* out);
 int hpe_debug_conv_stream1x1(const HpeConfig* cfg, int idx, int B, int concurrent, int residual);
 int hpe_debug_dual(hpe_ctx* ctx, int idx2c, const float* t2_dev, const float* x_dev, int B, float* y_dev, void* stream);
+int hpe_debug_stream_chain(hpe_ctx* ctx, int idx2c, const float* t2_dev, const float* x_dev, int B, float* t3_dev, float* u1_dev, int slab8,
+                           int rows, void* stream);
 int hpe_debug_gemm(hpe_ctx* ctx, const float* x_dev, const float* wt_dev, int M, int N, int K, int w_rows, int tile,
                    const float* residual_dev, int relu, float* y_dev, void* stream);
 int hpe_debug_maxpool(const float* x_dev, int B, int H, int C, float* y_dev, void* stream);
```
